# khaotik/DaNet-Tensorflow

Hardware: AMD Instinct MI355X
Metric: mixture-seconds/s (train step) (higher is better)
Workload: dtype f32; 1 GPU; cfg2: synthetic 8 kHz 2-spk, FFT 256/64 (129 bins), T=128, 3x300 BiLSTM, E=20, anchor estimator (A=6), dot-softmax, B=32/GPU; global_batch=32, parallelism=dp1, grad_allreduce_bytes=27619696, grad_allreduce_schedule=0

## Files before the change

danet-tensorflow_amd/_build.py:

```python
import collections
import glob
import os
import subprocess
import sys
from concurrent.futures import ThreadPoolExecutor

HERE = os.path.dirname(os.path.abspath(__file__))
CSRC = os.path.join(HERE, 'csrc')
INCLUDE = os.path.join(os.path.dirname(HERE), 'include')
ARCH = 'gfx950'
HIPCC = os.environ.get('HIPCC', '/opt/rocm/bin/hipcc')
FLAGS = ['--offload-arch=' + ARCH, '-O3', '-std=c++17', '-fPIC', '-fvisibility=hidden', '-I' + INCLUDE,
         '-I' + CSRC, '-Wno-unused-result']
FLAGS += os.environ.get('DANET_BUILD_DEFS', '').split()

Library = collections.namedtuple('Library', 'out src_dir headers')


def _extension(name, *more_headers):
    src_dir = os.path.join(CSRC, name)
    return Library(os.path.join(CSRC, 'libdanet_%s_hip.so' % name), src_dir,
                   (os.path.join(INCLUDE, 'danet_%s_hip.h' % name),) + more_headers)


def _shared(*names):
    return tuple(os.path.join(CSRC, n + '.h') for n in names)


CORE = Library(os.path.join(CSRC, 'libdanet_hip.so'), CSRC, (os.path.join(CSRC, '*.h'), os.path.join(INCLUDE, '*.h')))
CONV = _extension('conv', os.path.join(CSRC, 'conv', '*.h'), *_shared('ext_core'))
DROPOUT = _extension('dropout', *_shared('ext_core'))
PREP = _extension('prep', *_shared('ext_core'))
MIX = _extension('mix', *_shared('ext_core', 'ragged_rows', 'sumsq_f64'))
SPEED = _extension('speed', *_shared('ext_core', 'ragged_rows'))
LIBRARIES = (CORE, CONV, DROPOUT, PREP, MIX, SPEED)
LIB, CONV_LIB, DROPOUT_LIB, PREP_LIB, MIX_LIB, SPEED_LIB = (spec.out for spec in LIBRARIES)
REVERB = _extension('reverb', *_shared('ext_core', 'ragged_rows'))
LATER_LIBRARIES = (REVERB,)
REVERB_LIB = REVERB.out
METRIC = _extension('metric', *_shared('wave_metric', 'ext_core'))
NOISE = _extension('noise', *_shared('ext_core'))
LEVEL = _extension('level', *_shared('ext_core', 'ragged_rows'))
WAVLOSS = _extension('wavloss', *_shared('wave_metric', 'ext_core'))
GCLIP = _extension('gclip', *_shared('ext_core', 'adam_one', 'sumsq_f64'))
DPCL = _extension('dpcl', *_shared('ext_core'))
NEVAL = _extension('neval', *_shared('wave_metric', 'ext_core'))
EXTENSIONS = (METRIC, NOISE, LEVEL, WAVLOSS, GCLIP, DPCL, NEVAL)
STITCH = _extension('stitch', *_shared('ext_core'))
BSS = _extension('bss', *_shared('ext_core'))
STOI = _extension('stoi', *_shared('ext_core'))
PHASE = _extension('phase', *_shared('ext_core', 'wave_metric'))
ONLINE = _extension('online', *_shared('ext_core'))
CAUSAL = _extension('causal', *_shared('ext_core'))
MORE_EXTENSIONS = (STITCH, BSS, STOI, PHASE, ONLINE, CAUSAL)
METRIC_LIB = METRIC.out
NOISE_LIB = NOISE.out
LEVEL_LIB = LEVEL.out
WAVLOSS_LIB = WAVLOSS.out
GCLIP_LIB = GCLIP.out
DPCL_LIB = DPCL.out
NEVAL_LIB = NEVAL.out
STITCH_LIB = STITCH.out
BSS_LIB = BSS.out
STOI_LIB = STOI.out
PHASE_LIB = PHASE.out
ONLINE_LIB = ONLINE.out
CAUSAL_LIB = CAUSAL.out


def _sources(src_dir):
    return sorted(f for f in os.listdir(src_dir) if f.endswith(('.hip', '.cpp')))


def _compile(src_dir, src, bdir, force, hdr_m, defs=()):
    obj = os.path.join(bdir, os.path.splitext(src)[0] + '.o')
    sp = os.path.join(src_dir, src)
    if (not force and os.path.exists(obj)
            and os.path.getmtime(obj) > max(os.path.getmtime(sp), hdr_m)):
        return obj, False
    cmd = [HIPCC] + FLAGS + list(defs) + ['-c', sp, '-o', obj]
    if src.endswith('.hip'):
        cmd[1:1] = ['-x', 'hip']
    r = subprocess.run(cmd, capture_output=True, text=True)
    if r.returncode != 0:
        raise RuntimeError('hipcc failed for %s:\n%s\n%s' % (src, r.stdout, r.stderr))
    return obj, True


def _compile_all(src_dir, bdir, force, hdr_m, defs=()):
    os.makedirs(bdir, exist_ok=True)
    srcs = _sources(src_dir)
    with ThreadPoolExecutor(max_workers=min(8, len(srcs))) as ex:
        return list(ex.map(lambda s: _compile(src_dir, s, bdir, force, hdr_m, defs), srcs))


def _link(objs, out, src_dir):
    cmd = [HIPCC, '--offload-arch=' + ARCH, '-shared', '-fPIC',
           '-Wl,--version-script=' + os.path.join(src_dir, 'exports.map'), '-o', out] + objs
    r = subprocess.run(cmd, capture_output=True, text=True)
    if r.returncode != 0:
        raise RuntimeError('link failed:\n%s\n%s' % (r.stdout, r.stderr))


def _build_spec(spec, force, verbose):
    hdr_m = max((os.path.getmtime(h) for pattern in spec.headers for h in glob.glob(pattern)), default=0.0)
    res = _compile_all(spec.src_dir, os.path.join(spec.src_dir, 'build'), force, hdr_m)
    objs = [o for o, _ in res]
    rebuilt = any(r for _, r in res)
    if rebuilt or not os.path.exists(spec.out):
        _link(objs, spec.out, spec.src_dir)
    if verbose:
        print('%s: %s (%d objects, %s)' % (
            os.path.basename(spec.out), spec.out, len(objs), 'rebuilt' if rebuilt else 'up to date'))
    return spec.out


def _build_library(spec, force, verbose):
    return _build_spec(spec, force, verbose)


def build(force=False, verbose=True):
    for spec in LIBRARIES + LATER_LIBRARIES:
        _build_library(spec, force, verbose)
    return LIB


def build_all(force=False, verbose=True):
    build(force, verbose)
    for spec in EXTENSIONS + MORE_EXTENSIONS:
        _build_spec(spec, force, verbose)
    return [spec.out for spec in LIBRARIES + LATER_LIBRARIES + EXTENSIONS + MORE_EXTENSIONS]


def build_conv(force=False, verbose=True):
    return _build_library(CONV, force, verbose)


def build_dropout(force=False, verbose=True):
    return _build_library(DROPOUT, force, verbose)


def build_prep(force=False, verbose=True):
    return _build_library(PREP, force, verbose)


def build_mix(force=False, verbose=True):
    return _build_library(MIX, force, verbose)


def build_speed(force=False, verbose=True):
    return _build_library(SPEED, force, verbose)


def build_reverb(force=False, verbose=True):
    return _build_library(REVERB, force, verbose)


def build_metric(force=False, verbose=True):
    return _build_spec(METRIC, force, verbose)


def build_noise(force=False, verbose=True):
    return _build_spec(NOISE, force, verbose)


def build_level(force=False, verbose=True):
    return _build_spec(LEVEL, force, verbose)


def build_wavloss(force=False, verbose=True):
    return _build_spec(WAVLOSS, force, verbose)


def build_gclip(force=False, verbose=True):
    return _build_spec(GCLIP, force, verbose)


def build_dpcl(force=False, verbose=True):
    return _build_spec(DPCL, force, verbose)


def build_neval(force=False, verbose=True):
    return _build_spec(NEVAL, force, verbose)


def build_stitch(force=False, verbose=True):
    return _build_spec(STITCH, force, verbose)


def build_bss(force=False, verbose=True):
    return _build_spec(BSS, force, verbose)


def build_stoi(force=False, verbose=True):
    return _build_spec(STOI, force, verbose)


def build_phase(force=False, verbose=True):
    return _build_spec(PHASE, force, verbose)


def build_online(force=False, verbose=True):
    return _build_spec(ONLINE, force, verbose)


def build_causal(force=False, verbose=True):
    return _build_spec(CAUSAL, force, verbose)


def build_variant(name, defs):
    out = os.path.join(CSRC, 'libdanet_hip_%s.so' % name)
    res = _compile_all(CSRC, os.path.join(CSRC, 'build_' + name), True, 0.0, defs)
    _link([o for o, _ in res], out, CSRC)
    return out


def build_trace():
    return build_variant('trace', ['-DDANET_LSTM_TRACE'])


if __name__ == '__main__':
    if '--trace' in sys.argv:
        print(build_trace())
    elif '--variant' in sys.argv:
        i = sys.argv.index('--variant')
        print(build_variant(sys.argv[i + 1], sys.argv[i + 2:]))
    else:
        build_all(force='--force' in sys.argv)
```

danet-tensorflow_amd/_lib.py:

```python
import collections
import ctypes
import os
import threading

import torch

_CSRC = os.path.join(os.path.dirname(os.path.abspath(__file__)), 'csrc')

c_int, c_i64, c_f32, c_sz, c_p, c_u32 = (ctypes.c_int, ctypes.c_int64, ctypes.c_float,
                                         ctypes.c_size_t, ctypes.c_void_p, ctypes.c_uint32)
c_f64 = ctypes.c_double


class GemmPack(ctypes.Structure):
    _fields_ = [('src', c_p), ('stride_n', ctypes.c_longlong), ('stride_k', ctypes.c_longlong),
                ('N', c_int), ('K', c_int), ('out', c_p), ('out_bytes', c_sz)]


class GemmProblem(ctypes.Structure):
    _fields_ = [('A', c_p), ('lda', c_int), ('B', c_p), ('ldb', c_int), ('C', c_p), ('ldc', c_int),
                ('M', c_int), ('N', c_int), ('bias', c_p), ('beta', c_f32)]


PROTOTYPES = {
# ... 103 lines not shown
                                    c_u32, c_u32]),
}

PREP_PROTOTYPES = {
    'danet_prep_abi_version': (c_int, []),
    'danet_prep_last_error': (ctypes.c_char_p, []),
    'danet_prep_num_frames': (c_int, [c_i64, c_int, c_int]),
    'danet_prep_workspace_bytes': (c_sz, [c_int]),
    'danet_prep_stft_plan': (c_int, [c_p, c_int, c_p, c_p, c_sz]),
    'danet_prep_stft_batch': (c_int, [c_p, c_int, c_p, c_i64, c_p, c_int, c_int, c_int, c_int, c_int, c_p, c_p,
                                      c_p, c_i64]),
}

MIX_PROTOTYPES = {
    'danet_mix_abi_version': (c_int, []),
    'danet_mix_last_error': (ctypes.c_char_p, []),
    'danet_mix_workspace_bytes': (c_sz, [c_int, c_i64]),
    'danet_mix_power': (c_int, [c_p, c_int, c_p, c_i64, c_p, c_p, c_i64, c_p, c_p, c_sz]),
    'danet_mix_scale_c64': (c_int, [c_p, c_int, c_int, c_int, c_p, c_i64, c_p]),
}

SPEED_PROTOTYPES = {
    'danet_speed_abi_version': (c_int, []),
    'danet_speed_last_error': (ctypes.c_char_p, []),
    'danet_speed_out_len': (c_i64, [c_i64, c_int]),
    'danet_speed_resample': (c_int, [c_p, c_int, c_p, c_i64, c_p, c_p, c_p, c_i64]),
}

REVERB_PROTOTYPES = {
    'danet_reverb_abi_version': (c_int, []),
    'danet_reverb_last_error': (ctypes.c_char_p, []),
    'danet_reverb_apply': (c_int, [c_p, c_int, c_p, c_i64, c_p, c_p, c_int, c_p, c_i64]),
}

METRIC_PROTOTYPES = {
    'danet_metric_abi_version': (c_int, []),
    'danet_metric_last_error': (ctypes.c_char_p, []),
    'danet_metric_workspace_bytes': (c_sz, [c_int, c_int, c_int, c_int, c_int]),
    'danet_metric_synth': (c_int, [c_p, c_int, c_int, c_int, c_int, c_int, c_p, c_p, c_p, c_p]),
    'danet_metric_gram': (c_int, [c_p, c_int, c_int, c_i64, c_p, c_p]),
    'danet_metric_si_sdr': (c_int, [c_p, c_int, c_int, c_p, c_p, c_p, c_p]),
}

NOISE_PROTOTYPES = {
    'danet_noise_abi_version': (c_int, []),
    'danet_noise_last_error': (ctypes.c_char_p, []),
    'danet_noise_frontend_fwd': (c_int, [c_p, c_int, c_int, c_i64, c_p, c_p, c_p, c_p, c_p, c_p, c_p, c_p]),
}

LEVEL_PROTOTYPES = {
    'danet_level_abi_version': (c_int, []),
    'danet_level_last_error': (ctypes.c_char_p, []),
    'danet_level_workspace_bytes': (c_sz, [c_int, c_i64]),
    'danet_level_activity': (c_int, [c_p, c_int, c_p, c_i64, c_p, c_p, c_i64, c_f64, c_i64, c_p, c_p, c_p, c_sz]),
}

WAVLOSS_PROTOTYPES = {
    'danet_wavloss_abi_version': (c_int, []),
    'danet_wavloss_last_error': (ctypes.c_char_p, []),
    'danet_wavloss_fwd': (c_int, [c_p, c_int, c_int, c_p, c_p, c_p, c_p, c_p, c_p, c_p]),
    'danet_wavloss_bwd': (c_int, [c_p, c_int, c_int, c_int, c_int, c_int, c_p, c_p, c_p, c_p, c_p, c_p, c_p]),
}

GCLIP_PROTOTYPES = {
    'danet_gclip_abi_version': (c_int, []),
    'danet_gclip_last_error': (ctypes.c_char_p, []),
    'danet_gclip_partials': (c_int, [c_i64]),
    'danet_gclip_sumsq': (c_int, [c_p, c_i64, c_p, c_p, c_int]),
    'danet_gclip_adam_step': (c_int, [c_p, c_i64, c_p, c_p, c_p, c_p, c_f32, c_f32, c_f32, c_f32, c_f32, c_f32, c_int,
                                      c_f64, c_p, c_int, c_p]),
}

DPCL_PROTOTYPES = {
    'danet_dpcl_abi_version': (c_int, []),
    'danet_dpcl_last_error': (ctypes.c_char_p, []),
    'danet_dpcl_chunks': (c_int, [c_i64]),
    'danet_dpcl_workspace_bytes': (c_sz, [c_int, c_i64, c_int, c_int]),
    'danet_dpcl_stats': (c_int, [c_p, c_int, c_i64, c_int, c_int, c_p, c_p, c_p, c_sz]),
    'danet_dpcl_finalize': (c_int, [c_p, c_int, c_i64, c_int, c_int, c_p, c_sz, c_p, c_f32, c_p, c_p, c_p, c_p, c_p]),
    'danet_dpcl_bwd': (c_int, [c_p, c_int, c_i64, c_int, c_int, c_p, c_p, c_p, c_p, c_p, c_f32, c_p]),
}

NEVAL_PROTOTYPES = {
    'danet_neval_abi_version': (c_int, []),
    'danet_neval_last_error': (ctypes.c_char_p, []),
    'danet_neval_workspace_bytes': (c_sz, [c_int, c_int, c_int, c_int, c_int]),
    'danet_neval_synth': (c_int, [c_p, c_int, c_int, c_int, c_int, c_int, c_p, c_p, c_p, c_p, c_p, c_p]),
    'danet_neval_gram': (c_int, [c_p, c_int, c_int, c_i64, c_p, c_p]),
    'danet_neval_si_sdr': (c_int, [c_p, c_int, c_int, c_p, c_p, c_p, c_p]),
}

STITCH_PROTOTYPES = {
    'danet_stitch_abi_version': (c_int, []),
    'danet_stitch_last_error': (ctypes.c_char_p, []),
    'danet_stitch_chunks': (c_int, [c_int, c_int, c_int]),
    'danet_stitch_workspace_bytes': (c_sz, [c_int, c_int, c_int, c_int, c_int]),
    'danet_stitch_affinity': (c_int, [c_p, c_int, c_int, c_int, c_int, c_int, c_p, c_p, c_sz]),
    'danet_stitch_assign': (c_int, [c_p, c_int, c_int, c_int, c_int, c_int, c_p, c_sz, c_p, c_p]),
    'danet_stitch_merge': (c_int, [c_p, c_int, c_int, c_int, c_int, c_int, c_p, c_p, c_p, c_p, c_p]),
}

BSS_PROTOTYPES = {
    'danet_bss_abi_version': (c_int, []),
    'danet_bss_last_error': (ctypes.c_char_p, []),
    'danet_bss_workspace_bytes': (c_sz, [c_int, c_int, c_int]),
    'danet_bss_xcorr': (c_int, [c_p, c_int, c_int, c_i64, c_int, c_p, c_p, c_p, c_p]),
    'danet_bss_systems': (c_int, [c_p, c_int, c_int, c_int, c_p, c_p, c_p, c_p, c_p, c_p]),
    'danet_bss_chol_solve': (c_int, [c_p, c_int, c_int, c_int, c_p, c_p, c_p]),
    'danet_bss_finalize': (c_int, [c_p, c_int, c_int, c_int, c_p, c_p, c_p, c_p, c_p, c_p, c_p, c_int, c_int,
                                   c_p, c_p, c_p, c_p]),
}

STOI_PROTOTYPES = {
    'danet_stoi_abi_version': (c_int, []),
    'danet_stoi_last_error': (ctypes.c_char_p, []),
    'danet_stoi_workspace_bytes': (c_sz, [c_int, c_int, c_i64, c_int, c_int]),
    'danet_stoi_resample': (c_int, [c_p, c_int, c_int, c_i64, c_int, c_int, c_p, c_p, c_p]),
    'danet_stoi_frames': (c_int, [c_p, c_int, c_int, c_i64, c_p, c_p, c_p, c_p, c_p, c_p, c_p]),
    'danet_stoi_bands': (c_int, [c_p, c_int, c_int, c_i64, c_p, c_p, c_p, c_p, c_p, c_p, c_p]),
    'danet_stoi_segments': (c_int, [c_p, c_int, c_int, c_int, c_p, c_p, c_p]),
    'danet_stoi_finalize': (c_int, [c_p, c_int, c_int, c_int, c_p, c_p, c_p, c_int, c_int, c_p, c_p, c_p, c_p, c_p]),
}

PHASE_PROTOTYPES = {
    'danet_phase_abi_version': (c_int, []),
    'danet_phase_last_error': (ctypes.c_char_p, []),
    'danet_phase_workspace_bytes': (c_sz, [c_int, c_int, c_int, c_int, c_int]),
    'danet_phase_init': (c_int, [c_p, c_int, c_int, c_int, c_int, c_int, c_int, c_p, c_p, c_p, c_p, c_p]),
    'danet_phase_synth': (c_int, [c_p, c_int, c_int, c_int, c_int, c_int, c_p, c_p, c_p]),
    'danet_phase_project': (c_int, [c_p, c_int, c_int, c_int, c_int, c_int, c_p, c_p, c_p, c_p]),
}

ONLINE_PROTOTYPES = {
    'danet_online_abi_version': (c_int, []),
    'danet_online_last_error': (ctypes.c_char_p, []),
    'danet_online_state_bytes': (c_sz, [c_int, c_int]),
    'danet_online_init': (c_int, [c_p, c_int, c_int, c_int, c_p, c_p]),
    'danet_online_scan': (c_int, [c_p, c_int, c_int, c_int, c_int, c_int, c_int, c_f64, c_int, c_i64, c_f64, c_p, c_p,
                                  c_p, c_p]),
    'danet_online_separate': (c_int, [c_p, c_int, c_int, c_int, c_int, c_int, c_int, c_p, c_p, c_p, c_p]),
}

CAUSAL_PROTOTYPES = {
    'danet_causal_abi_version': (c_int, []),
    'danet_causal_last_error': (ctypes.c_char_p, []),
    'danet_causal_center_fwd': (c_int, [c_p, c_int, c_int, c_int, c_p, c_int, c_int, c_p, c_int, c_int, c_p]),
    'danet_causal_center_bwd': (c_int, [c_p, c_int, c_int, c_int, c_p, c_int, c_int, c_p, c_int, c_int]),
    'danet_causal_lstm_ws_bytes': (c_sz, [c_int, c_int, c_int, c_int]),
    'danet_causal_lstm_block': (c_int, [c_p, c_int, c_int, c_int, c_int, c_int, c_p, c_int, ctypes.POINTER(c_p),
                                        ctypes.POINTER(c_p), c_p, c_p, c_p, c_int, c_p, c_sz]),
    'danet_causal_project': (c_int, [c_p, c_int, c_int, c_int, c_p, c_int, c_p, c_int, c_p, c_int]),
}

Library = collections.namedtuple('Library', 'name so path_var handle_var prototypes abi prefix needs')
CONV_ABI_VERSION = DROPOUT_ABI_VERSION = PREP_ABI_VERSION = MIX_ABI_VERSION = SPEED_ABI_VERSION = 1
REVERB_ABI_VERSION = 1

CORE = Library('', 'libdanet_hip.so', 'LIB_PATH', '_lib', PROTOTYPES, 7, 'danet_',
               'the HIP extension is required')
CONV = Library('conv', 'libdanet_conv_hip.so', 'CONV_LIB_PATH', '_conv', CONV_PROTOTYPES, CONV_ABI_VERSION,
               'danet_conv_', 'the conv-bilstm-v1 encoder needs the HIP extension library')
DROPOUT = Library('dropout', 'libdanet_dropout_hip.so', 'DROPOUT_LIB_PATH', '_dropout', DROPOUT_PROTOTYPES,
                  DROPOUT_ABI_VERSION, 'danet_dropout_', 'DROPOUT_KEEP_PROB < 1 needs the HIP extension library')
PREP = Library('prep', 'libdanet_prep_hip.so', 'PREP_LIB_PATH', '_prep', PREP_PROTOTYPES, PREP_ABI_VERSION,
               'danet_prep_', 'the wavdir dataset needs the HIP extension library')
MIX = Library('mix', 'libdanet_mix_hip.so', 'MIX_LIB_PATH', '_mix', MIX_PROTOTYPES, MIX_ABI_VERSION,
              'danet_mix_', 'MIX_SNR_RANGE / MIX_LEVEL_RANGE need the HIP extension library')
SPEED = Library('speed', 'libdanet_speed_hip.so', 'SPEED_LIB_PATH', '_speed', SPEED_PROTOTYPES, SPEED_ABI_VERSION,
                'danet_speed_', 'SPEED_PERTURB_RANGE needs the HIP extension library')
REVERB = Library('reverb', 'libdanet_reverb_hip.so', 'REVERB_LIB_PATH', '_reverb', REVERB_PROTOTYPES,
                 REVERB_ABI_VERSION, 'danet_reverb_', 'REVERB_RT60_MAX needs the HIP extension library')
LIBRARIES = (CORE, CONV, DROPOUT, PREP, MIX)
ALL_LIBRARIES = LIBRARIES + (SPEED,)
LATER_LIBRARIES = (REVERB,)
METRIC_ABI_VERSION = 1
METRIC = Library('metric', 'libdanet_metric_hip.so', 'METRIC_LIB_PATH', '_metric', METRIC_PROTOTYPES,
                 METRIC_ABI_VERSION, 'danet_metric_', 'EVAL_SI_SDR needs the HIP extension library')
NOISE_ABI_VERSION = 1
NOISE = Library('noise', 'libdanet_noise_hip.so', 'NOISE_LIB_PATH', '_noise', NOISE_PROTOTYPES,
                NOISE_ABI_VERSION, 'danet_noise_', 'NOISE_DIR needs the HIP extension library')
LEVEL_ABI_VERSION = 1
LEVEL = Library('level', 'libdanet_level_hip.so', 'LEVEL_LIB_PATH', '_level', LEVEL_PROTOTYPES,
                LEVEL_ABI_VERSION, 'danet_level_', 'MIX_LEVEL_MEASURE needs the HIP extension library')
WAVLOSS_ABI_VERSION = 1
WAVLOSS = Library('wavloss', 'libdanet_wavloss_hip.so', 'WAVLOSS_LIB_PATH', '_wavloss', WAVLOSS_PROTOTYPES,
                  WAVLOSS_ABI_VERSION, 'danet_wavloss_', 'TRAIN_LOSS = "si-sdr" needs the HIP extension library')
GCLIP_ABI_VERSION = 1
GCLIP = Library('gclip', 'libdanet_gclip_hip.so', 'GCLIP_LIB_PATH', '_gclip', GCLIP_PROTOTYPES,
                GCLIP_ABI_VERSION, 'danet_gclip_', 'GRAD_CLIP_NORM needs the HIP extension library')
DPCL_ABI_VERSION = 1
DPCL = Library('dpcl', 'libdanet_dpcl_hip.so', 'DPCL_LIB_PATH', '_dpcl', DPCL_PROTOTYPES,
               DPCL_ABI_VERSION, 'danet_dpcl_', 'DPCL_WEIGHT needs the HIP extension library')
NEVAL_ABI_VERSION = 1
NEVAL = Library('neval', 'libdanet_neval_hip.so', 'NEVAL_LIB_PATH', '_neval', NEVAL_PROTOTYPES,
                NEVAL_ABI_VERSION, 'danet_neval_', 'NOISE_EVAL_DIR with EVAL_SI_SDR needs the HIP extension library')
STITCH_ABI_VERSION = 1
STITCH = Library('stitch', 'libdanet_stitch_hip.so', 'STITCH_LIB_PATH', '_stitch', STITCH_PROTOTYPES,
                 STITCH_ABI_VERSION, 'danet_stitch_', 'INFER_CHUNK_LEN needs the HIP extension library')
EXTENSIONS = (METRIC, NOISE, LEVEL, WAVLOSS, GCLIP, DPCL, NEVAL)
BSS_ABI_VERSION = 1
BSS = Library('bss', 'libdanet_bss_hip.so', 'BSS_LIB_PATH', '_bss', BSS_PROTOTYPES,
              BSS_ABI_VERSION, 'danet_bss_', 'EVAL_BSS_SDR needs the HIP extension library')
STOI_ABI_VERSION = 1
STOI = Library('stoi', 'libdanet_stoi_hip.so', 'STOI_LIB_PATH', '_stoi', STOI_PROTOTYPES,
               STOI_ABI_VERSION, 'danet_stoi_', 'EVAL_STOI needs the HIP extension library')
PHASE_ABI_VERSION = 1
PHASE = Library('phase', 'libdanet_phase_hip.so', 'PHASE_LIB_PATH', '_phase', PHASE_PROTOTYPES,
                PHASE_ABI_VERSION, 'danet_phase_', 'PHASE_REFINE_ITERS needs the HIP extension library')
ONLINE_ABI_VERSION = 1
ONLINE = Library('online', 'libdanet_online_hip.so', 'ONLINE_LIB_PATH', '_online', ONLINE_PROTOTYPES,
                 ONLINE_ABI_VERSION, 'danet_online_', 'the "online" estimator needs the HIP extension library')
CAUSAL_ABI_VERSION = 1
CAUSAL = Library('causal', 'libdanet_causal_hip.so', 'CAUSAL_LIB_PATH', '_causal', CAUSAL_PROTOTYPES,
                 CAUSAL_ABI_VERSION, 'danet_causal_', 'the lstm-causal encoder and streaming inference need the HIP '
                 'extension library')
MORE_EXTENSIONS = (STITCH, BSS, STOI, PHASE, ONLINE, CAUSAL)

LIB_PATH = os.environ.get('DANET_LIB_PATH') or os.path.join(_CSRC, CORE.so)
CONV_LIB_PATH = os.path.join(_CSRC, CONV.so)
DROPOUT_LIB_PATH = os.path.join(_CSRC, DROPOUT.so)
PREP_LIB_PATH = os.path.join(_CSRC, PREP.so)
MIX_LIB_PATH = os.path.join(_CSRC, MIX.so)
SPEED_LIB_PATH = os.path.join(_CSRC, SPEED.so)
REVERB_LIB_PATH = os.path.join(_CSRC, REVERB.so)
METRIC_LIB_PATH = os.path.join(_CSRC, METRIC.so)
NOISE_LIB_PATH = os.path.join(_CSRC, NOISE.so)
LEVEL_LIB_PATH = os.path.join(_CSRC, LEVEL.so)
WAVLOSS_LIB_PATH = os.path.join(_CSRC, WAVLOSS.so)
GCLIP_LIB_PATH = os.path.join(_CSRC, GCLIP.so)
DPCL_LIB_PATH = os.path.join(_CSRC, DPCL.so)
NEVAL_LIB_PATH = os.path.join(_CSRC, NEVAL.so)
STITCH_LIB_PATH = os.path.join(_CSRC, STITCH.so)
BSS_LIB_PATH = os.path.join(_CSRC, BSS.so)
STOI_LIB_PATH = os.path.join(_CSRC, STOI.so)
PHASE_LIB_PATH = os.path.join(_CSRC, PHASE.so)
ONLINE_LIB_PATH = os.path.join(_CSRC, ONLINE.so)
CAUSAL_LIB_PATH = os.path.join(_CSRC, CAUSAL.so)
_lib = _conv = _dropout = _prep = _mix = _speed = _reverb = _metric = _noise = _level = _wavloss = _gclip = _dpcl = None
_neval = _stitch = _bss = _stoi = _phase = _online = _causal = None
_lock = threading.Lock()


class DanetHipError(RuntimeError):
    pass


def _load(spec, loaded=None):
    g = globals()
    if g[spec.handle_var] is None:
        with _lock:
            if g[spec.handle_var] is None:
                path = g[spec.path_var]
                if not os.path.exists(path):
                    raise DanetHipError(
                        '%s not found at %s -- %s (there is no CPU fallback); build it with '
                        '`python -c "import __graft_entry__ as g; g.build()"`' % (spec.so, path, spec.needs))
                lib = ctypes.CDLL(path, mode=ctypes.RTLD_LOCAL)
                for name, (res, args) in spec.prototypes.items():
                    fn = getattr(lib, name)
                    fn.restype = res
                    fn.argtypes = args
                if getattr(lib, spec.prefix + 'abi_version')() != spec.abi:
                    raise DanetHipError('%s ABI version mismatch' % spec.so)
                g[spec.handle_var] = lib
                if loaded is not None:
                    loaded()
    return g[spec.handle_var]


def _check(spec, rc):
    msg = getattr(_load(spec), spec.prefix + 'last_error')()
    raise DanetHipError('%s error %d: %s' % (spec.so[:-3], rc, msg.decode() if msg else '?'))


def bytes_or_raise(nbytes, check):
    if nbytes == ctypes.c_size_t(-1).value:
        check(-1)
    return nbytes


def load():
    if _lib is not None:
        return _lib
    return _load(CORE, apply_env_options)


def load_conv():
    if _conv is not None:
        return _conv
    return _load(CONV)


def conv_check(rc):
    if rc != 0:
        _check(CONV, rc)


def conv_ws_bytes(op, desc):
    return bytes_or_raise(load_conv().danet_conv_workspace_bytes(op, ctypes.byref(desc)), conv_check)


def load_dropout():
    if _dropout is not None:
        return _dropout
    return _load(DROPOUT)


def dropout_check(rc):
    if rc != 0:
        _check(DROPOUT, rc)


def load_prep():
    if _prep is not None:
        return _prep
    return _load(PREP)


def prep_check(rc):
    if rc != 0:
        _check(PREP, rc)


def load_mix():
    if _mix is not None:
        return _mix
    return _load(MIX)


def mix_check(rc):
    if rc != 0:
        _check(MIX, rc)


def load_speed():
    if _speed is not None:
        return _speed
    return _load(SPEED)


def speed_check(rc):
    if rc != 0:
        _check(SPEED, rc)


def load_reverb():
    if _reverb is not None:
        return _reverb
    return _load(REVERB)


def reverb_check(rc):
    if rc != 0:
        _check(REVERB, rc)


def load_metric():
    if _metric is not None:
        return _metric
    return _load(METRIC)


def metric_check(rc):
    if rc != 0:
        _check(METRIC, rc)


def load_noise():
    if _noise is not None:
        return _noise
    return _load(NOISE)


def noise_check(rc):
    if rc != 0:
        _check(NOISE, rc)


def load_level():
    if _level is not None:
        return _level
    return _load(LEVEL)


def level_check(rc):
    if rc != 0:
        _check(LEVEL, rc)


def load_wavloss():
    if _wavloss is not None:
        return _wavloss
    return _load(WAVLOSS)


def wavloss_check(rc):
    if rc != 0:
        _check(WAVLOSS, rc)


def load_gclip():
    if _gclip is not None:
        return _gclip
    return _load(GCLIP)


def gclip_check(rc):
    if rc != 0:
        _check(GCLIP, rc)


def load_dpcl():
    if _dpcl is not None:
        return _dpcl
    return _load(DPCL)


def dpcl_check(rc):
    if rc != 0:
        _check(DPCL, rc)


def load_neval():
    if _neval is not None:
        return _neval
    return _load(NEVAL)


def neval_check(rc):
    if rc != 0:
        _check(NEVAL, rc)


def load_stitch():
    if _stitch is not None:
        return _stitch
    return _load(STITCH)


def stitch_check(rc):
    if rc != 0:
        _check(STITCH, rc)


def load_bss():
    if _bss is not None:
        return _bss
    return _load(BSS)


def bss_check(rc):
    if rc != 0:
        _check(BSS, rc)


def load_stoi():
    if _stoi is not None:
        return _stoi
    return _load(STOI)


def stoi_check(rc):
    if rc != 0:
        _check(STOI, rc)


def load_phase():
    if _phase is not None:
        return _phase
    return _load(PHASE)


def phase_check(rc):
    if rc != 0:
        _check(PHASE, rc)


def load_online():
    if _online is not None:
        return _online
    return _load(ONLINE)


def online_check(rc):
    if rc != 0:
        _check(ONLINE, rc)


def load_causal():
    if _causal is not None:
        return _causal
    return _load(CAUSAL)


def causal_check(rc):
    if rc != 0:
        _check(CAUSAL, rc)


_expert = None
_expert_seen = set()


def expert(name, default):
    global _expert
    if _expert is None:
        _expert = {}
        for item in os.environ.get('DANET_EXPERT', '').split(','):
            if item.strip():
                k, _, v = item.partition('=')
                _expert[k.strip().lower()] = v.strip()
    _expert_seen.add(name.lower())
    v = _expert.get(name.lower())
    if v is None:
        return default
    if isinstance(default, bool):
        return v not in ('0', 'false', 'no', '')
    return type(default)(v)


USER_OPTIONS = ('lstm_fwd_fused', 'lstm_spin_limit', 'lstm_fault_inject')


def option_names():
    lib = _lib
    return [lib.danet_option_name(i).decode() for i in range(lib.danet_option_count())]


def apply_env_options():
    lib = _lib
    lib.danet_reset_options()
    for name in option_names():
        v = os.environ.get('DANET_' + name.upper()) if name in USER_OPTIONS else None
        if v is None or v.strip() == '':
            v = expert(name, '')
        if v != '':
            check(lib.danet_set_option(name.encode(), int(v)))
    unknown = sorted(set(_expert or {}) - _expert_seen)
    if unknown:
        import warnings
        warnings.warn('DANET_EXPERT: unknown setting(s) %s (known: the lower-case constants of ops.py / model.py '
                      'that call _lib.expert(), and the library options %s)' % (unknown, option_names()))


def set_option(name, value):
    check(load().danet_set_option(name.encode(), int(value)))


def get_option(name):
    v = c_int(0)
    check(load().danet_get_option(name.encode(), ctypes.byref(v)))
    return v.value


def check(rc):
    if rc != 0:
        _check(CORE, rc)


(WS_ISTFT, WS_GEMM, WS_GEMM_STREAMK, WS_COLSUM, WS_LSTM, WS_ATTRACTOR_TRUTH, WS_ATTRACTOR_ANCHOR,
 WS_SEPARATE_BWD, WS_SEPARATE_PIT, WS_SEPARATE_PIT_RECORDS, WS_PIT_MSE, WS_CENTER_MEAN,
 WS_GEMM_X6, WS_GEMM_PACK, WS_GEMM_X6_TN, WS_SEPARATE_PIT_GRAD) = range(16)


def ws_bytes(op, *dims):
    arr = (c_i64 * len(dims))(*[int(d) for d in dims])
    return bytes_or_raise(load().danet_workspace_bytes(op, arr, len(dims)), check)


def ptr(t):
    if t is None:
        return None
    return t.data_ptr()


def stream():
    return torch.cuda.current_stream().cuda_stream


_ws = {}


def workspace(nbytes, device, tag=None):
    key = (device.index if device.index is not None else torch.cuda.current_device(),
           torch.cuda.current_stream().cuda_stream, tag)
    t = _ws.get(key)
    if t is None or t.numel() < nbytes:
        t = torch.zeros(max(int(nbytes), 1 << 20), dtype=torch.uint8, device=device)
        _ws[key] = t
    return t


_prof = None
_prof_only = None
_prof_on = True


def profile_start(only=None):
    global _prof, _prof_only
    if torch.cuda.is_available():
        prepare_timing(64)
    _prof = {}
    _prof_only = set(only) if only else None


def profile_enable(flag):
    global _prof_on
    _prof_on = bool(flag)


def profile_stop():
    global _prof
    p, _prof = _prof, None
    torch.cuda.synchronize()
    out = {}
    for label, evs in (p or {}).items():
        out[label] = (len(evs), sum(a.elapsed_time(b) for a, b in evs))
    return out


ATTACHED_LABELS = frozenset(('lstm_fwd', 'lstm_bwd'))
_aux_stream = None
_event_pool = []


def _timing_event():
    global _aux_stream
    if _event_pool:
        return _event_pool.pop()
    return _timing_event_new()


def prepare_timing(n=384):
    made = False
    while len(_event_pool) < n:
        _event_pool.append(_timing_event_new())
        made = True
    if made:
        torch.cuda.synchronize()


def _timing_event_new():
    global _aux_stream
    if _aux_stream is None:
        _aux_stream = torch.cuda.Stream()
    e = torch.cuda.Event(enable_timing=True)
    e.record(_aux_stream)
    return e


class timed(object):
    __slots__ = ('label', 'tag', 'a', 'b')

    def __init__(self, label, tag=None):
        self.label, self.tag = label, tag

    def __enter__(self):
        self.a = self.b = None
        if _prof is not None and _prof_on and (_prof_only is None or self.label in _prof_only):
            if self.label in ATTACHED_LABELS:
                self.a, self.b = _timing_event(), _timing_event()
                check(load().danet_next_launch_events(self.a.cuda_event, self.b.cuda_event))
            else:
                self.a = torch.cuda.Event(enable_timing=True)
                self.a.record()
        return self

    def __exit__(self, *exc):
        if self.a is not None and _prof is not None:
            b = self.b
            if b is None:
                b = torch.cuda.Event(enable_timing=True)
                b.record()
            _prof.setdefault(self.label, []).append((self.a, b))
            if self.tag:
                _prof.setdefault(self.label + ':' + self.tag, []).append((self.a, b))
        return False
```

danet-tensorflow_amd/csrc/gemm_x6.hip:

```cpp
#include "common.h"
#include <hip/hip_ext.h>
#include <atomic>
#include "danet_hip.h"
#include "options.h"

typedef __bf16 bf16x8 __attribute__((ext_vector_type(8)));
typedef uint32_t u32x4 __attribute__((ext_vector_type(4)));
typedef uint32_t u32x2 __attribute__((ext_vector_type(2)));

#define XBN 128
#define X6_OOB 0xfffffff0u
#define XBK 16

template <int MI> struct X6Geo {
  static constexpr int BM = 64 * MI;
  static constexpr int IMG = BM * XBK * 2;
  static constexpr int STAGE = 3 * IMG;
  static constexpr int LDC_T = XBN + 4;
  static constexpr int EPI = 32 * MI * LDC_T * 4;
  static constexpr int SMEM = 3 * STAGE > EPI ? 3 * STAGE : EPI;
  static constexpr int NS = 12 * MI;
  static constexpr int WG_PER_CU = MI == 2 ? 2 : 1;
};

// ... 749 lines not shown
      *reinterpret_cast<f32x4*>(o) = v;
    }
  }
}

template <bool RAGGED>
__global__ __launch_bounds__(256, 2) void gemm_x6_tn_kernel(X6TArgs g) {
  extern __shared__ __attribute__((aligned(16))) char xsm[];
  if ((int)blockIdx.x < g.ntail) {
    x6t_tail(g, (int)blockIdx.x, xsm);
    return;
  }
  const int tid = threadIdx.x, lane = tid & 63, wave = __builtin_amdgcn_readfirstlane(tid >> 6);
  const int wm = wave >> 1, wn = wave & 1;
  const int item = x6_xcd_item((int)blockIdx.x - g.ntail, (int)gridDim.x - g.ntail);
  const int z = item / g.tiles;
  const int t = item % g.tiles;
  int pi = 0;
#pragma unroll
  for (int i = 1; i < X6T_MAX_PROBLEMS; ++i)
    if (i < g.nprob && t >= g.p[i].tile0) pi = i;
  const X6TProblem& q = g.p[pi];
  const int tl = t - q.tile0;
  const int m0 = (tl / q.tiles_n) * 128, n0 = (tl % q.tiles_n) * 128;
  const int M = q.Mmain, N = q.N, K = g.K;

  const int nkt = (K + 15) / 16;
  const int per = (nkt + g.splitk - 1) / g.splitk;
  const int kt0 = z * per, kt1 = min(nkt, kt0 + per);

  X6TCtx c;
  {
    const float* ab = q.A + m0;
    const float* bb = q.B + n0;
    c.rsa = __builtin_amdgcn_make_buffer_rsrc(const_cast<float*>(ab), 0, (int)(((size_t)(K - 1) * q.lda + ((M - m0 + 3) & ~3)) * 4), 0x00020000);
    c.rsb = __builtin_amdgcn_make_buffer_rsrc(const_cast<float*>(bb), 0, (int)(((size_t)(K - 1) * q.ldb + ((N - n0 + 3) & ~3)) * 4), 0x00020000);
  }
  c.lda = q.lda; c.ldb = q.ldb; c.K = K; c.kt1 = kt1; c.mrem = M - m0; c.nrem = N - n0;
  const int kr = lane >> 4, mq = lane & 15;
  c.krow = 4 * wave + kr;
  c.mq4 = 4 * mq;
#pragma unroll
  for (int li = 0; li < 4; ++li) {
    const int col = c.mq4 + (li & 1) * 64;
    c.lvo[li] = col < (li < 2 ? c.mrem : c.nrem) ? (unsigned)(c.krow * (li < 2 ? c.lda : c.ldb) + col) * 4u : X6_OOB;
  }
  c.woff = (wave * 8 + (mq >> 2)) * 128 + ((kr + (mq >> 2)) & 3) * 32 + (mq & 3) * 8;
  {
    const int i16 = lane & 15, mbit = (lane >> 4) & 1, kh = lane >> 5;
#pragma unroll
    for (int i = 0; i < 2; ++i) {
      const int ba = (wm * 64 + i * 32 + 16 * mbit) >> 4, bb = (wn * 64 + i * 32 + 16 * mbit) >> 4;
      c.roffa[i] = (2 * kh * 8 + ba) * 128 + (((i16 >> 2) + ba) & 3) * 32 + (i16 & 3) * 8;
      c.roffb[i] = (2 * kh * 8 + bb) * 128 + (((i16 >> 2) + bb) & 3) * 32 + (i16 & 3) * 8;
    }
  }
  const int fi = lane & 31, kb = lane >> 5;

  f32x16 acc[2][2];
#pragma unroll
  for (int i = 0; i < 2; ++i)
#pragma unroll
    for (int j = 0; j < 2; ++j)
#pragma unroll
      for (int r = 0; r < 16; ++r) acc[i][j][r] = 0.f;

  if (kt0 < kt1) {
    f32x4 R0[4], R1[4];
    bf16x8 faA[3][2], fbA[3][2], faB[3][2], fbB[3][2];
    x6t_load_tile<RAGGED>(c, kt0, R0); x6t_load_tile<RAGGED>(c, kt0 + 1, R1);
    x6t_store_tile(xsm, c, R0); x6t_store_tile(xsm + TSTAGE, c, R1);
    x6t_load_tile<RAGGED>(c, kt0 + 2, R0); x6t_load_tile<RAGGED>(c, kt0 + 3, R1);
    __syncthreads();
    x6t_frags(xsm, c, faA, fbA);
    int kt = kt0, srd = 1, swr = 2;
#define X6T_STEP(SRD, SWR, R, FAC, FBC, FAN, FBN)                                                    \
    { x6t_step<RAGGED, SRD, SWR>(c, xsm, kt, srd, swr, acc, R, FAC, FBC, FAN, FBN);                  \
      __syncthreads();                                                                               \
      ++kt; }
#define X6T_STEP_RT(R, FAC, FBC, FAN, FBN)                                                           \
    { x6t_step<RAGGED, -1, -1>(c, xsm, kt, srd, swr, acc, R, FAC, FBC, FAN, FBN);                    \
      __syncthreads();                                                                               \
      ++kt; srd = swr; swr = swr == 2 ? 0 : swr + 1; }
    while (kt + 5 < kt1) {
      X6T_STEP(1, 2, R0, faA, fbA, faB, fbB)
      X6T_STEP(2, 0, R1, faB, fbB, faA, fbA)
      X6T_STEP(0, 1, R0, faA, fbA, faB, fbB)
      X6T_STEP(1, 2, R1, faB, fbB, faA, fbA)
      X6T_STEP(2, 0, R0, faA, fbA, faB, fbB)
      X6T_STEP(0, 1, R1, faB, fbB, faA, fbA)
    }
    while (kt + 1 < kt1) {
      X6T_STEP_RT(R0, faA, fbA, faB, fbB)
      X6T_STEP_RT(R1, faB, fbB, faA, fbA)
    }
    if (kt < kt1) X6T_STEP_RT(R0, faA, fbA, faB, fbB)
#undef X6T_STEP
#undef X6T_STEP_RT
  }

  const bool sliced = g.splitk > 1;
  float* __restrict__ dst = sliced ? g.slab + (size_t)z * g.slab_stride + q.slab_off : q.C;
  const int ldc = sliced ? N : q.ldc;
  const float beta = sliced ? 0.f : q.beta;
  const bool vec = (ldc % 4 == 0) && (((uintptr_t)dst & 15) == 0) && (n0 + 128 <= N);
  if (vec) {
    float* ct = reinterpret_cast<float*>(xsm);
    constexpr int LDC_T = 132;
#pragma unroll
    for (int half = 0; half < 2; ++half) {
      __syncthreads();
      if (wm == half) {
#pragma unroll
        for (int i = 0; i < 2; ++i)
#pragma unroll
          for (int j = 0; j < 2; ++j)
#pragma unroll
            for (int r = 0; r < 16; ++r)
              ct[(i * 32 + (r & 3) + 8 * (r >> 2) + 4 * kb) * LDC_T + wn * 64 + j * 32 + fi] = acc[i][j][r];
      }
      __syncthreads();
#pragma unroll
      for (int it = 0; it < 8; ++it) {
        const int rr = (tid >> 5) + 8 * it, c4 = tid & 31;
        const int row = m0 + half * 64 + rr;
        if (row < M) {
          f32x4* o = reinterpret_cast<f32x4*>(dst + (size_t)row * ldc + n0 + c4 * 4);
          f32x4 v = *reinterpret_cast<const f32x4*>(&ct[rr * LDC_T + c4 * 4]);
          if (beta != 0.f) v += *o;
          *o = v;
        }
      }
    }
    return;
  }
#pragma unroll
  for (int i = 0; i < 2; ++i)
#pragma unroll
    for (int j = 0; j < 2; ++j) {
      const int col = n0 + wn * 64 + j * 32 + fi;
#pragma unroll
      for (int r = 0; r < 16; ++r) {
        const int row = m0 + wm * 64 + i * 32 + (r & 3) + 8 * (r >> 2) + 4 * kb;
        if (row < M && col < N) {
          float* o = dst + (size_t)row * ldc + col;
          *o = acc[i][j][r] + (beta != 0.f ? *o : 0.f);
        }
      }
    }
}

__global__ __launch_bounds__(256) void gemm_x6_tn_reduce_kernel(X6TArgs g) {
  const X6TProblem& q = g.p[blockIdx.y];
  const int M = q.M, N = q.N, ldc = q.ldc;
  const float beta = q.beta;
  const float* __restrict__ slab = g.slab + q.slab_off;
  const int64_t n4 = (int64_t)M * N / 4;
  for (int64_t i = (int64_t)blockIdx.x * 256 + threadIdx.x; i < n4; i += (int64_t)gridDim.x * 256) {
    f32x4 v = reinterpret_cast<const f32x4*>(slab)[i];
    for (int s = 1; s < g.splitk; ++s) v += reinterpret_cast<const f32x4*>(slab + (size_t)s * g.slab_stride)[i];
    const int64_t e = i * 4;
    f32x4* o = reinterpret_cast<f32x4*>(q.C + (size_t)(e / N) * ldc + (e % N));
    if (beta != 0.f) v += *o;
    *o = v;
  }
}

#ifdef X6T_FORCE_S
static int x6t_splitk(int tiles, int K) { return tiles >= 100 ? X6T_FORCE_S : x6_slices(tiles, cdiv(K, 16), 16, 8); }
#else
static int x6t_splitk(int tiles, int K) { return x6_slices(tiles, cdiv(K, 16), 16, 8, 0.045); }
#endif
static int x6t_main_rows(int M, int N) {
  const int tail = M % 128;
  return (M > 128 && tail >= 1 && tail <= X6T_TAIL_MAX && N % 4 == 0) ? M - tail : M;
}
size_t dn_ws_gemm_x6_tn(long long sum_mn, int tiles, int K) {
  const int s = x6t_splitk(tiles, K);
  return s > 1 ? (size_t)s * (size_t)sum_mn * sizeof(float) : 0;
}

extern "C" int danet_gemm_x6_tn_grouped(danet_stream_t stream_, int K, int nprob, const danet_gemm_problem_t* probs,
                                        void* ws, size_t ws_bytes) {
  hipStream_t stream = (hipStream_t)stream_;
  DANET_CHECK_ARG(probs && nprob >= 1 && nprob <= X6T_MAX_PROBLEMS, "gemm_x6_tn: 1..%d problems", X6T_MAX_PROBLEMS);
  DANET_CHECK_ARG(K > 0, "gemm_x6_tn: non-positive K %d", K);
  X6TArgs g;
  int tiles = 0;
  long long sum_mn = 0;
  bool slicable = true, ragged = false;
  for (int i = 0; i < nprob; ++i) {
    const danet_gemm_problem_t& q = probs[i];
    DANET_CHECK_ARG(q.M > 0 && q.N > 0 && q.A && q.B && q.C, "gemm_x6_tn: bad problem %d", i);
    DANET_CHECK_ARG(q.bias == nullptr && (q.beta == 0.f || q.beta == 1.f), "gemm_x6_tn: no bias; beta 0 or 1");
    DANET_CHECK_ARG(q.lda >= q.M && q.ldb >= q.N && q.ldc >= q.N, "gemm_x6_tn: leading dimension too small");
    if (q.lda % 4 || q.ldb % 4 || ((((uintptr_t)q.A | (uintptr_t)q.B)) & 15) != 0) {
      danet_set_error("gemm_x6_tn: lda / ldb must be multiples of 4 and A / B 16-byte aligned (problem %d)", i);
      return DANET_ERR_UNSUPPORTED;
    }
    DANET_CHECK_ARG((long long)K * q.lda < (1ll << 29) && (long long)K * q.ldb < (1ll << 29),
                    "gemm_x6_tn: an operand spans 2 GiB or more");
    X6TProblem& p = g.p[i];
    p.A = q.A; p.B = q.B; p.C = q.C; p.lda = q.lda; p.ldb = q.ldb; p.ldc = q.ldc; p.M = q.M; p.N = q.N;
    p.beta = q.beta;
    p.Mmain = ((((uintptr_t)q.C) & 15) == 0 && q.ldc % 4 == 0) ? x6t_main_rows(q.M, q.N) : q.M;
    p.tiles_n = cdiv(q.N, 128);
    p.tile0 = tiles;
    p.slab_off = sum_mn;
    tiles += cdiv(p.Mmain, 128) * p.tiles_n;
    sum_mn += (long long)q.M * q.N;
    ragged = ragged || (p.Mmain % 2 != 0) || (q.N % 2 != 0);
    slicable = slicable && q.N % 4 == 0 && q.ldc % 4 == 0 && (((uintptr_t)q.C) & 15) == 0 && ((long long)q.M * q.N) % 4 == 0;
  }
  for (int i = nprob; i < X6T_MAX_PROBLEMS; ++i) g.p[i] = g.p[0];
  g.nprob = nprob; g.K = K; g.tiles = tiles;
  int s = slicable ? x6t_splitk(tiles, K) : 1;
  g.splitk = s;
  g.slab_stride = sum_mn;
  g.slab = (float*)ws;
  g.ntail = 0;
  for (int i = 0; i < nprob; ++i)
    if (g.p[i].Mmain < g.p[i].M) g.ntail += cdiv(g.p[i].N, 64) * s;
  if (s > 1) {
    const size_t need = (size_t)s * (size_t)sum_mn * sizeof(float);
    if (!ws || ws_bytes < need || ((uintptr_t)ws & 15) != 0) {
      danet_set_error("gemm_x6_tn: workspace %zu < %zu (or not 16-B aligned)", ws_bytes, need);
      return DANET_ERR_WORKSPACE;
    }
  }
  static std::atomic<unsigned long long> done[2];
  dim3 grid((unsigned)(tiles * s + g.ntail)), block(256);
  if (ragged) {
    DANET_CHECK_HIP(x6_set_lds((const void*)gemm_x6_tn_kernel<true>, X6T_SMEM_BYTES, done[1]));
    gemm_x6_tn_kernel<true><<<grid, block, X6T_SMEM_BYTES, stream>>>(g);
  } else {
    DANET_CHECK_HIP(x6_set_lds((const void*)gemm_x6_tn_kernel<false>, X6T_SMEM_BYTES, done[0]));
    gemm_x6_tn_kernel<false><<<grid, block, X6T_SMEM_BYTES, stream>>>(g);
  }
  DANET_CHECK_LAUNCH();
  if (s > 1) {
    long long most = 0;
    for (int i = 0; i < nprob; ++i) most = max(most, (long long)probs[i].M * probs[i].N / 4);
    dim3 rgrid((unsigned)min((long long)1024, (most + 255) / 256), (unsigned)nprob);
    gemm_x6_tn_reduce_kernel<<<rgrid, block, 0, stream>>>(g);
    DANET_CHECK_LAUNCH();
  }
  return DANET_OK;
}
```

danet-tensorflow_amd/csrc/lstm.hip:

```cpp
#include "common.h"
#include "options.h"
#include <hip/hip_ext.h>
#include <atomic>
#include <type_traits>
#include <stdlib.h>

void dn_take_launch_events(hipEvent_t* start, hipEvent_t* stop);
#define DN_LAUNCH_EV(K_, GRID_, BLOCK_, LDS_, STREAM_, ARGS_)                                        \
  do {                                                                                               \
    if (ev_start || ev_stop)                                                                         \
      hipExtLaunchKernelGGL(K_, dim3(GRID_), dim3(BLOCK_), LDS_, STREAM_, ev_start, ev_stop, 0, ARGS_); \
    else K_<<<GRID_, BLOCK_, LDS_, STREAM_>>>(ARGS_);                                                \
  } while (0)

#define LSTM_UNITS_FWD 8
#define SPIN_LIMIT (1u << 20)
#define FWD_CH 5
#define SENTINEL 0xFFFFFFFFu

#define RLX_AGENT __ATOMIC_RELAXED, __HIP_MEMORY_SCOPE_AGENT

typedef unsigned v4u __attribute__((__vector_size__(16)));

__device__ __forceinline__ v4u load_sc1_b128(__amdgpu_buffer_rsrc_t r, unsigned off) {
// ... 1197 lines not shown
      dp += gstep;
    }
    if constexpr (!SHADOW) { gp += gstep; cp += cstep; dyp += ystep; }
    TRACE(5);
  }
  shadow_store(T - 1);
  if constexpr (PRE) { if (othr) db_add(); }
  if (a.dbslab != nullptr && tw == 0) {
    float* dbt = &atile[SSTORE ? (T & 1) * ATILE : 0];
    __syncthreads();
    if (othr) {
      float* ap = &dbt[orow * LDA + oj];
      ap[0] = dbacc[0]; ap[U] = dbacc[1]; ap[2 * U] = dbacc[2]; ap[3 * U] = dbacc[3];
    }
    __syncthreads();
    if (tid < 4 * U) {
      float v = 0.f;
#pragma unroll
      for (int rr = 0; rr < 16; ++rr) v += dbt[rr * LDA + tid];
      const int gate = tid / U, j = tid % U;
      if (u0 + j < H) a.dbslab[(size_t)cl * (4 * H) + gate * H + u0 + j] = v;
    }
  }
}

__global__ __launch_bounds__(256) void lstm_db_reduce_kernel(
    const float* __restrict__ dbslab, float* db0, float* db1, int G, int H4, float beta) {
  const int dir = blockIdx.y;
  float* db = dir ? db1 : db0;
  const int q4 = H4 / 4;
  for (int j = blockIdx.x * 256 + threadIdx.x; j < q4; j += gridDim.x * 256) {
    f32x4 v = {0.f, 0.f, 0.f, 0.f};
    for (int g = 0; g < G; ++g)
      v += reinterpret_cast<const f32x4*>(dbslab + (size_t)(dir * G + g) * H4)[j];
    f32x4* o = reinterpret_cast<f32x4*>(db) + j;
    if (beta != 0.f) v += *o;
    *o = v;
  }
}

__global__ __launch_bounds__(256) void multi_fill_kernel(FillArgs a) {
  fill_share(a, (unsigned long long)blockIdx.x * 256 + threadIdx.x, (unsigned long long)gridDim.x * 256);
}

struct FillList {
  FillArgs a;
  FillList() { a.nseg = 0; }
  bool full() const { return a.nseg >= FILL_MAXSEG; }
  void add(void* p, size_t bytes, unsigned value) {
    a.ptr[a.nseg] = p; a.n16[a.nseg] = bytes / 16; a.value[a.nseg] = value; ++a.nseg;
  }
  hipError_t launch(hipStream_t stream) {
    unsigned long long tot = 0;
    for (int i = 0; i < a.nseg; ++i) tot += a.n16[i];
    unsigned long long blocks = (tot + 256 * 4 - 1) / (256 * 4);
    if (blocks > 2048) blocks = 2048;
    if (blocks < 1) blocks = 1;
    multi_fill_kernel<<<(unsigned)blocks, 256, 0, stream>>>(a);
    return hipGetLastError();
  }
};

struct LstmPlan { int MT, G, P, KP, NW, UN; size_t lds; };

int dn_num_cus() {
  static std::atomic<int> n{0};
  int c = n.load(std::memory_order_relaxed);
  if (c) return c;
  int dev = 0, v = 0;
  if (hipGetDevice(&dev) == hipSuccess &&
      hipDeviceGetAttribute(&v, hipDeviceAttributeMultiprocessorCount, dev) == hipSuccess && v > 0) {
    n.store(v, std::memory_order_relaxed);
    return v;
  }
  (void)hipGetLastError();
  return 256;
}

static LstmPlan make_plan(int B, int H, int ndir) {
  LstmPlan pl;
  pl.UN = LSTM_UNITS_FWD;
  pl.P = cdiv(H, pl.UN);
  pl.KP = cdiv(H, 16) * 16;
  pl.MT = (ndir * cdiv(B, 16) * pl.P > dn_num_cus()) ? 2 : 1;
  if (B > 4) {
    const int want = danet_opt(OPT_LSTM_FWD_UN);
    const bool fits12 = ndir * cdiv(B, 16) * cdiv(H, 12) <= dn_num_cus();
    if ((want == 12 || (want != 8 && pl.MT == 2)) && fits12) {
      pl.UN = 12; pl.P = cdiv(H, 12); pl.MT = 1;
    }
  }
  pl.G = cdiv(B, 16 * pl.MT);
  pl.NW = 4;
  { const int ngw = cdiv(pl.KP / 16, pl.NW), nbw = (ngw + 1) / 2;
    pl.lds = (((size_t)pl.NW * 16 * pl.MT * (4 * pl.UN + 1) + 3) & ~(size_t)3) * sizeof(float) +
             (size_t)pl.NW * (nbw > 3 ? nbw - 3 : 0) * 3 * (4 * pl.UN / 16) * 64 * 16; }
  return pl;
}

struct RsPlan { bool ok; int U, G, P, S, NT, NTW, NI, D; size_t ring_bytes; };
static RsPlan make_rs_plan(int B, int H, int ndir, int U) {
  RsPlan r;
  r.U = U; r.G = cdiv(B, 16); r.P = cdiv(H, U);
  r.NT = cdiv(r.P * U, 16); r.D = 3;
  r.NI = cdiv(r.P, 512 / (4 * U));
  const int ncl = ndir * r.G;
  int smax = dn_num_cus() / (ncl * r.P);
  if (smax > r.NT) smax = r.NT;
  r.S = smax;
  for (int sv = 1; sv <= smax; ++sv)
    if (cdiv(r.NT, sv) <= 8) { r.S = sv; break; }
  { const int es = danet_opt(OPT_LSTM_BWD_S);
    if (es >= 1 && es <= smax) r.S = es; }
  r.NTW = r.S > 0 ? cdiv(cdiv(r.NT, r.S), 8) : 99;
  r.ring_bytes = (size_t)r.D * ncl * r.P * r.NT * 1024;
  r.ok = (H % 4 == 0) && smax >= 1 && r.NTW <= 5 && r.NI <= RS_NI_MAX &&
         r.ring_bytes < 0xFFFFFFF0ull;
  return r;
}
static RsPlan choose_rs_plan(int B, int H, int ndir) {
  RsPlan none; none.ok = false; none.ring_bytes = 0;
  const int pin = danet_opt(OPT_LSTM_BWD_U);
  if (!pin && H > 384) {
    const RsPlan r = make_rs_plan(B, H, ndir, 16);
    if (r.ok) return r;
  }
  RsPlan best = none;
  int best_cost = 1 << 30;
  for (int U = 8; U <= 32; U *= 2) {
    if (pin && pin != U) continue;
    RsPlan r = make_rs_plan(B, H, ndir, U);
    if (!r.ok) continue;
    const int cost = cdiv(cdiv(r.NT, r.S), 4) * U;
    if (cost < best_cost) { best = r; best_cost = cost; }
  }
  return best;
}
static size_t ring_offset(int T) { return (64 + TRACE_BYTES(T) + 255) / 256 * 256; }
static unsigned spin_limit_env() {
  const long v = danet_opt(OPT_LSTM_SPIN_LIMIT);
  return v >= 256 ? (unsigned)v : SPIN_LIMIT;
}
static int fault_env() { return danet_opt(OPT_LSTM_FAULT_INJECT) == 1; }

size_t dn_ws_lstm(int T, int B, int H, int ndir) {
  size_t ring = 0;
  for (int U = 8; U <= 32; U *= 2) {
    RsPlan r = make_rs_plan(B, H, ndir, U);
    if (r.ok && r.ring_bytes > ring) ring = r.ring_bytes;
  }
  return align_up(ring_offset(T) + ring, 256) + align_up((size_t)ndir * cdiv(B, 16) * 4 * H * sizeof(float), 256);
}

static int lstm_check_common(int T, int B, int H, int ndir, void* ws, size_t ws_bytes) {
  DANET_CHECK_ARG(T > 0 && B > 0 && H > 0, "lstm: non-positive shape");
  DANET_CHECK_ARG(ndir == 1 || ndir == 2, "lstm: ndir must be 1 or 2");
  if (H % 4 != 0) {
    danet_set_error("lstm: H=%d must be a multiple of 4", H);
    return DANET_ERR_UNSUPPORTED;
  }
  if (!ws || ((uintptr_t)ws & 15) != 0 || ws_bytes < dn_ws_lstm(T, B, H, ndir)) {
    danet_set_error("lstm: workspace too small or not 16-B aligned");
    return DANET_ERR_WORKSPACE;
  }
  return DANET_OK;
}

static int prefill_fwd_segments(FillList& fl, hipStream_t stream, int T, int B, int ldy, int n,
                                float* const* ypads, void* const* wss) {
  const size_t blk = (size_t)B * ldy * sizeof(float);
  for (int i = 0; i < n; ++i) {
    DANET_CHECK_ARG(ypads[i] && ((uintptr_t)ypads[i] & 15) == 0, "lstm_prefill: ypad %d null / misaligned", i);
    if (fl.a.nseg + 4 > FILL_MAXSEG) { DANET_CHECK_HIP(fl.launch(stream)); fl = FillList(); }
    if (wss && wss[i]) fl.add(wss[i], 64 + TRACE_BYTES(T), 0u);
    fl.add((char*)ypads[i] + blk, (size_t)T * blk, SENTINEL);
    fl.add(ypads[i], blk, 0u);
    fl.add((char*)ypads[i] + (size_t)(T + 1) * blk, blk, 0u);
  }
  return DANET_OK;
}

static int prefill_bwd_segments(FillList& fl, hipStream_t stream, int T, const RsPlan& rs, int n,
                                void* const* wss) {
  for (int i = 0; i < n; ++i) {
    DANET_CHECK_ARG(wss[i] && ((uintptr_t)wss[i] & 15) == 0, "lstm_prefill: ws %d null / misaligned", i);
    if (fl.a.nseg + 2 > FILL_MAXSEG) { DANET_CHECK_HIP(fl.launch(stream)); fl = FillList(); }
    fl.add(wss[i], 64 + TRACE_BYTES(T), 0u);
    fl.add((char*)wss[i] + ring_offset(T), rs.ring_bytes, 1u);
  }
  return DANET_OK;
}

extern "C" int danet_lstm_fwd_prefill(danet_stream_t stream_, int T, int B, int ldy, int n,
                                      float* const* ypads, void* const* wss) {
  hipStream_t stream = (hipStream_t)stream_;
  DANET_CHECK_ARG(T > 0 && B > 0 && ldy > 0 && ldy % 4 == 0 && n > 0 && ypads, "lstm_fwd_prefill: bad argument");
  FillList fl;
  const int rc = prefill_fwd_segments(fl, stream, T, B, ldy, n, ypads, wss);
  if (rc) return rc;
  if (fl.a.nseg) DANET_CHECK_HIP(fl.launch(stream));
  return DANET_OK;
}

extern "C" int danet_lstm_train_prefill(danet_stream_t stream_, int T, int B, int H, int ndir, int ldy,
                                        int n, float* const* ypads, void* const* fwd_wss,
                                        void* const* bwd_wss) {
  hipStream_t stream = (hipStream_t)stream_;
  DANET_CHECK_ARG(T > 0 && B > 0 && H > 0 && (ndir == 1 || ndir == 2) && ldy > 0 && ldy % 4 == 0 && n > 0 &&
                  ypads && bwd_wss, "lstm_train_prefill: bad argument");
  const RsPlan rs = choose_rs_plan(B, H, ndir);
  if (!rs.ok) {
    danet_set_error("lstm_train_prefill: B=%d H=%d outside the reduce-scatter geometry", B, H);
    return DANET_ERR_UNSUPPORTED;
  }
  FillList fl;
  int rc = prefill_fwd_segments(fl, stream, T, B, ldy, n, ypads, fwd_wss);
  if (rc) return rc;
  rc = prefill_bwd_segments(fl, stream, T, rs, n, bwd_wss);
  if (rc) return rc;
  if (fl.a.nseg) DANET_CHECK_HIP(fl.launch(stream));
  return DANET_OK;
}

extern "C" int danet_encoder_prologue(danet_stream_t stream_, int B, int T, int D, const float* in,
                                      int in_layout, int ld_in, float* out, int out_layout, int ld_out,
                                      float* mean, int H, int ndir, int ldy, int n, float* const* ypads,
                                      void* const* fwd_wss, void* const* bwd_wss) {
  hipStream_t stream = (hipStream_t)stream_;
  DANET_CHECK_ARG(T > 0 && B > 0 && H > 0 && (ndir == 1 || ndir == 2) && ldy > 0 && ldy % 4 == 0 && n > 0 &&
                  ypads, "encoder_prologue: bad argument");
  FillList fl;
  int rc;
  const bool one = 4 * n + (bwd_wss ? 2 * n : 0) <= FILL_MAXSEG;
  if (bwd_wss) {
    const RsPlan rs = choose_rs_plan(B, H, ndir);
    if (!rs.ok) {
      danet_set_error("encoder_prologue: B=%d H=%d outside the reduce-scatter geometry", B, H);
      return DANET_ERR_UNSUPPORTED;
    }
    rc = prefill_fwd_segments(fl, stream, T, B, ldy, n, ypads, fwd_wss);
    if (rc) return rc;
    rc = prefill_bwd_segments(fl, stream, T, rs, n, bwd_wss);
    if (rc) return rc;
  } else {
    rc = prefill_fwd_segments(fl, stream, T, B, ldy, n, ypads, fwd_wss);
    if (rc) return rc;
  }
  bool taken = false;
  rc = dn_center(stream, B, T, D, in, in_layout, ld_in, out, out_layout, ld_out, mean,
                 one && fl.a.nseg ? &fl.a : nullptr, &taken);
  if (rc) return rc;
  if (!taken && fl.a.nseg) DANET_CHECK_HIP(fl.launch(stream));
  return DANET_OK;
}

extern "C" int danet_lstm_fwd(danet_stream_t stream_, int T, int B, int H, int ndir,
                              const float* gx_f, const float* gx_b,
                              const float* Wh_f, const float* Wh_b, int ldw,
                              float* ypad, int ldy, float* gates_f, float* gates_b,
                              float* cell_f, float* cell_b, void* ws, size_t ws_bytes,
                              int32_t* status, int flags) {
  hipEvent_t ev_start, ev_stop;
  dn_take_launch_events(&ev_start, &ev_stop);
  hipStream_t stream = (hipStream_t)stream_;
  int rc = lstm_check_common(T, B, H, ndir, ws, ws_bytes);
  if (rc) return rc;
  DANET_CHECK_ARG(gx_f && Wh_f && ypad && gates_f && cell_f, "lstm_fwd: null pointer");
  DANET_CHECK_ARG(ndir == 1 || (gx_b && Wh_b && gates_b && cell_b), "lstm_fwd: null bwd pointer");
  DANET_CHECK_ARG(ldy >= ndir * H && ldy % 4 == 0 && ldw >= 4 * H, "lstm_fwd: bad ld");
  DANET_CHECK_ARG(((uintptr_t)ypad & 15) == 0, "lstm_fwd: ypad must be 16-B aligned");
  DANET_CHECK_ARG((size_t)(T + 2) * B * ldy * 4 < 0xFFFFFFF0ull, "lstm_fwd: ypad > 4 GiB");
  LstmPlan pl = make_plan(B, H, ndir);
  if (pl.lds > 160 * 1024) {
    danet_set_error("lstm_fwd: H=%d needs %zu B LDS", H, pl.lds);
    return DANET_ERR_UNSUPPORTED;
  }
  const int nblk = ndir * pl.G * pl.P;
  if (nblk > dn_num_cus()) {
    danet_set_error("lstm_fwd: %d workgroups exceed the %d CUs", nblk, dn_num_cus());
    return DANET_ERR_UNSUPPORTED;
  }
  LstmFwdArgs a;
  a.gx[0] = gx_f; a.gx[1] = gx_b; a.Wh[0] = Wh_f; a.Wh[1] = Wh_b;
  a.gates[0] = gates_f; a.gates[1] = gates_b; a.cell[0] = cell_f; a.cell[1] = cell_b;
  a.ypad = ypad; a.status = status ? (int*)status : (int*)ws;
  a.spin_limit = spin_limit_env(); a.fault = fault_env();
  a.T = T; a.B = B; a.H = H; a.ndir = ndir; a.ldy = ldy; a.ldw = ldw;
  a.P = pl.P; a.G = pl.G; a.KP = pl.KP;
  a.xmap = (danet_opt(OPT_LSTM_XMAP) >= 0 ? danet_opt(OPT_LSTM_XMAP) : 1);
  const size_t blk = (size_t)B * ldy * sizeof(float);
  if (!(flags & DANET_LSTM_PREFILLED)) {
    FillList fl;
    fl.add(ws, 64 + TRACE_BYTES(T), 0u);
    fl.add((char*)ypad + blk, (size_t)T * blk, SENTINEL);
    fl.add(ypad, blk, 0u);
    fl.add((char*)ypad + (size_t)(T + 1) * blk, blk, 0u);
    DANET_CHECK_HIP(fl.launch(stream));
  }
#define LAUNCH_FWD(MTV, NWV, UNV)                                                    \
  do {                                                                               \
    DANET_CHECK_HIP(hipFuncSetAttribute((const void*)lstm_fwd_kernel<MTV, NWV, UNV>,  \
        hipFuncAttributeMaxDynamicSharedMemorySize, (int)pl.lds));                   \
    DN_LAUNCH_EV((lstm_fwd_kernel<MTV, NWV, UNV>), nblk, 64 * NWV, pl.lds, stream, a); \
  } while (0)
  if (B <= 4 && H <= 16 * FWD_CH * 4 && danet_opt(OPT_LSTM_FWD_SMALL) != 0) {
    const size_t lds = ((size_t)pl.KP * 32 + (size_t)4 * 4 * 33) * sizeof(float);
// ... 194 lines not shown
```

danet-tensorflow_amd/csrc/workspace.cpp:

```cpp
#include <stddef.h>
#include <stdint.h>
#include "danet_hip.h"

extern "C" void danet_set_error(const char* fmt, ...);

size_t dn_ws_istft(int n_sig, int T, int N, int S);
size_t dn_ws_gemm(int M, int N, int K);
size_t dn_ws_gemm_streamk(int M, int N, int K);
size_t dn_ws_colsum(int M, int N);
size_t dn_ws_lstm(int T, int B, int H, int ndir);
size_t dn_ws_attractor_truth(int B, int C, int64_t N, int E);
size_t dn_ws_attractor_anchor(int B, int C, int64_t N, int E, int A);
size_t dn_ws_separate_bwd(int B, int C, int64_t N, int E);
size_t dn_ws_separate_pit(int B, int C, int64_t N, int E);
size_t dn_ws_separate_pit_records(int B, int64_t N);
size_t dn_ws_pit_mse(int B, int C, int64_t N);
int dn_center_mean_elems(int B);
size_t dn_ws_gemm_x6(int M, int N, int K1, int K2);
size_t dn_ws_gemm_pack(int N, int K);
size_t dn_ws_gemm_x6_tn(long long sum_mn, int tiles, int K);
size_t dn_ws_separate_pit_grad(int B, int C, int64_t N, int E);

extern "C" size_t danet_workspace_bytes(int op, const int64_t* d, int n) {
  static const int kDims[DANET_WS_COUNT] = {4, 3, 3, 2, 4, 4, 5, 4, 4, 2, 3, 1, 4, 2, 3, 4};
  if (op < 0 || op >= DANET_WS_COUNT || !d || n != kDims[op]) {
    danet_set_error("workspace_bytes: op %d takes %d dims, got %d", op,
                    (op >= 0 && op < DANET_WS_COUNT) ? kDims[op] : -1, n);
    return (size_t)-1;
  }
  for (int i = 0; i < n; ++i)
    if (d[i] < 0 || (d[i] > 0x7fffffff && !(i == 2 && op >= DANET_WS_ATTRACTOR_TRUTH) &&
                     !(i == 1 && op == DANET_WS_SEPARATE_PIT_RECORDS) &&
                     !(i == 0 && op == DANET_WS_GEMM_X6_TN))) {
      danet_set_error("workspace_bytes: dim %d of op %d out of range", i, op);
      return (size_t)-1;
    }
  switch (op) {
    case DANET_WS_ISTFT: return dn_ws_istft((int)d[0], (int)d[1], (int)d[2], (int)d[3]);
    case DANET_WS_GEMM: return dn_ws_gemm((int)d[0], (int)d[1], (int)d[2]);
    case DANET_WS_GEMM_STREAMK: return dn_ws_gemm_streamk((int)d[0], (int)d[1], (int)d[2]);
    case DANET_WS_COLSUM: return dn_ws_colsum((int)d[0], (int)d[1]);
    case DANET_WS_LSTM: return dn_ws_lstm((int)d[0], (int)d[1], (int)d[2], (int)d[3]);
    case DANET_WS_ATTRACTOR_TRUTH: return dn_ws_attractor_truth((int)d[0], (int)d[1], d[2], (int)d[3]);
    case DANET_WS_ATTRACTOR_ANCHOR:
      return dn_ws_attractor_anchor((int)d[0], (int)d[1], d[2], (int)d[3], (int)d[4]);
    case DANET_WS_SEPARATE_BWD: return dn_ws_separate_bwd((int)d[0], (int)d[1], d[2], (int)d[3]);
    case DANET_WS_SEPARATE_PIT: return dn_ws_separate_pit((int)d[0], (int)d[1], d[2], (int)d[3]);
    case DANET_WS_SEPARATE_PIT_RECORDS: return dn_ws_separate_pit_records((int)d[0], d[1]);
    case DANET_WS_PIT_MSE: return dn_ws_pit_mse((int)d[0], (int)d[1], d[2]);
    case DANET_WS_CENTER_MEAN: return (size_t)dn_center_mean_elems((int)d[0]) * sizeof(float);
    case DANET_WS_GEMM_X6: return dn_ws_gemm_x6((int)d[0], (int)d[1], (int)d[2], (int)d[3]);
    case DANET_WS_GEMM_PACK: return dn_ws_gemm_pack((int)d[0], (int)d[1]);
    case DANET_WS_GEMM_X6_TN: return dn_ws_gemm_x6_tn((long long)d[0], (int)d[1], (int)d[2]);
    case DANET_WS_SEPARATE_PIT_GRAD: return dn_ws_separate_pit_grad((int)d[0], (int)d[1], d[2], (int)d[3]);
  }
  return (size_t)-1;
}
```

danet-tensorflow_amd/model.py:

```python
import math
import os

import numpy as np
import torch

from .hparams import hparams
from . import _lib, ops
from . import modules
from . import ozers
from . import dist


class Model(object):

    def __init__(self, name='BaseModel', device=None, seed=1337, grad_schedule=None):
        self.grad_schedule = str(grad_schedule if grad_schedule is not None else
                                 os.environ.get('DANET_OVERLAP_ALLREDUCE', 'auto'))
        assert self.grad_schedule in ('0', 'tail', '1', 'auto'), self.grad_schedule
        self.schedule_decision = None
        self._auto = self.grad_schedule == 'auto'
        if self._auto:
            self.grad_schedule = '0'
        self.name = name
        self.device = torch.device(device if device is not None else
# ... 374 lines not shown

    def _auto_tick(self):
        n = self.step_count
        if n == self.AUTO_DECIDE_AT - 3:
            self._auto_ev = torch.cuda.Event(enable_timing=True)
            self._auto_ev.record()
        if n < self.AUTO_DECIDE_AT or self._auto_ev is None:
            return
        end = torch.cuda.Event(enable_timing=True)
        end.record()
        end.synchronize()
        step_ms = dist.allreduce_max_scalar(self._auto_ev.elapsed_time(end) / 3.0, self.device)
        ar_ms = dist.measure_allreduce_ms(self._grad_store.numel(), self.device)
        mode = dist.choose_schedule(ar_ms, step_ms)
        self.schedule_decision = dict(schedule=mode, allreduce_ms=round(ar_ms, 4), step_ms=round(step_ms, 4),
                                      ratio=round(ar_ms / step_ms, 5), threshold=dist.TAIL_RATIO,
                                      bucket_bytes=4 * self._grad_store.numel(), decided_at_step=n,
                                      world=dist.world_size())
        self._auto, self._auto_ev = False, None
        self._install_schedule(mode)

    @property
    def _early_adam(self):
        return self._early_adam_on

    @_early_adam.setter
    def _early_adam(self, on):
        self._early_adam_on = bool(on)
        if on and not self._early_hooked:
            ops.add_grad_ready_hook(self._grad_ready)
            self._early_hooked = True

    def _grad_ready(self, tag, params):
        if self.grad_clip_norm is not None:
            return
        if tag[0] != 'rest' or not self._early_adam or not self._in_step or self._early is not None:
            return
        rng = [self._offs.get(p.data_ptr()) for p in params]
        if any(r is None for r in rng):
            return
        if dist.is_dist():
            if not isinstance(self._buckets, dist.TailOverlap):
                return
            self._buckets.wait_launched()
        ranges = dist._complement(rng, self._flat_grad.numel())
        self.ozer.step(self.step_count + 1, self.learn_rate, clip=hparams.GRAD_CLIP_THRES,
                       grad_scale=1.0 / dist.world_size(), zero_grad=not self.keep_grads,
                       ranges=ranges)
        ops.repack_weights(self.device)
        self._early = (ranges, torch.cuda.current_stream(self.device))
        self.early_steps += 1

    def dropout_spec(self, keep):
        if self._dropout is None or self._dropout.keep != float(keep):
            self._dropout = ops.DropoutSpec(keep, self.seed & 0xffffffff, dist.rank(),
                                            self.step_base + self.step_count)
        return self._dropout

    def forward(self, s_src_signals, with_valid=False, with_train=True, fuse_heads=False,
                s_dropout_keep=1.0):
        B, E = hparams.BATCH_SIZE, hparams.EMBED_SIZE
        eps = float(hparams.EPS)
        if self._noise is None:
            fe = ops.frontend(s_src_signals)
        else:
            fe = ops.noise_frontend(s_src_signals, *self._noise)
        self._dropout = None
        if s_dropout_keep < 1.0:
            s_embed = self.encoder(fe['mix_log'], s_dropout_keep)
        else:
            s_embed = self.encoder(fe['mix_log'])
        s_embed_flat = s_embed.reshape(B, -1, E)
        out = dict(embed=s_embed, input=s_src_signals)
        phasor = fe['phasor']
        if with_train:
            s_attractors = self.estimator(
                s_embed, s_src_pwr=fe['src_pwr'], s_mix_pwr=fe['mix_pwr'])
            act = getattr(self.separator, 'ACT', None)
            if self.dpcl_weight is not None:
                ops.unshare_dembed(s_attractors)
            if self.train_loss == 'si-sdr':
                s_sep_pwr = self.separator(fe['mix_pwr'], s_attractors, s_embed_flat)
                loss, loss_idx = ops.si_sdr_loss(s_src_signals, s_sep_pwr, phasor)
                with torch.no_grad():
                    _mse, perms, idx, snr = ops.pit_mse_loss(
                        s_src_signals, s_sep_pwr.detach(), phasor, mode=0, eps=eps)
                out.update(attrs=s_attractors, sep_pwr=s_sep_pwr, loss=loss, SNR=snr,
                           perm_idx=idx, perms=perms, loss_perm_idx=loss_idx)
            elif fuse_heads and act is not None and not hparams.DEBUG and not with_valid:
                loss, perms, idx, snr = ops.separate_pit_loss(
                    fe['mix_pwr'], s_attractors, s_embed_flat, s_src_signals, phasor, act,
                    mode=0, eps=eps)
                out.update(attrs=s_attractors, loss=loss, SNR=snr, perm_idx=idx, perms=perms)
            else:
                s_sep_pwr = self.separator(fe['mix_pwr'], s_attractors, s_embed_flat)
                loss, perms, idx, snr = ops.pit_mse_loss(
                    s_src_signals, s_sep_pwr, phasor, mode=0, eps=eps)
                out.update(attrs=s_attractors, sep_pwr=s_sep_pwr, loss=loss, SNR=snr,
                           perm_idx=idx, perms=perms)
            if self.dpcl_weight is not None:
                out['loss'], out['dpcl'] = ops.dpcl_loss(s_embed_flat, fe['src_pwr'], out['loss'], self.dpcl_weight)
        if with_valid:
            if self.using_same_method and with_train:
                s_vattr, s_vsep = out['attrs'], out['sep_pwr']
            else:
                if self.valid_estimator.USE_TRUTH:
                    s_vattr = self.valid_estimator(
                        s_embed, s_src_pwr=fe['src_pwr'], s_mix_pwr=fe['mix_pwr'])
                else:
                    s_vattr = self.valid_estimator(s_embed, s_mix_pwr=fe['mix_pwr'])
                s_vsep = self._separate(fe['mix_pwr'], s_vattr, s_embed_flat)
            vloss, perms, vidx, vsnr = ops.pit_mse_loss(
                s_src_signals, s_vsep, phasor, mode=1, eps=eps)
            out.update(valid_attrs=s_vattr, sep_pwr_valid=s_vsep, valid_loss=vloss,
                       valid_SNR=vsnr, valid_perm_idx=vidx, perms=perms)
        out['phasor'] = phasor
        out['mix_pwr'] = fe['mix_pwr']
        return out

    def forward_noisy(self, s_src_signals, s_noise, s_noise_gain=None, **kw):
        self._noise = (s_noise, s_noise_gain)
        try:
            return self.forward(s_src_signals, **kw)
        finally:
            self._noise = None

    def debug_fetch(self, s_src_signals):
        with torch.no_grad():
            o = self.forward(s_src_signals)
            res = dict(embed=o['embed'], attrs=o['attrs'], input=s_src_signals,
                       output=ops.reattach_phase(o['sep_pwr'], o['phasor'], o['perm_idx']))
            for mod in (self.encoder, self.separator, self.estimator):
                res.update(getattr(mod, 'debug_fetches', {}) or {})
        return res

    def train_step(self, s_src_signals, sync_metrics=True, s_noise=None, s_noise_gain=None):
        ops.poll_status(self.device)
        if not self._grads_clean:
            self._flat_grad.zero_()
        chain = ops.heads_chain()
        chain.__enter__()
        try:
            if s_noise is None:
                out = self.forward(s_src_signals, fuse_heads=self.fuse_heads,
                                   s_dropout_keep=float(hparams.DROPOUT_KEEP_PROB))
            else:
                out = self.forward_noisy(s_src_signals, s_noise, s_noise_gain, fuse_heads=self.fuse_heads,
                                         s_dropout_keep=float(hparams.DROPOUT_KEEP_PROB))
        except BaseException:
            chain.__exit__(None, None, None)
            ops.drop_lazy(self.device)
            raise
        self._early, self._in_step = None, True
        self._grads_clean = False
        try:
            with ops.fast_backward():
                out['loss'].backward(self._one)
                ops.join_deferred()
                if self._buckets is not None:
                    grad_scale = self._buckets.finish()
                else:
                    grad_scale = dist.allreduce_grads_(
                        self._grad_store if dist.is_dist() else self._flat_grad)
        finally:
            self._in_step = False
            chain.__exit__(None, None, None)
            ops.join_deferred()
        self.step_count += 1
        ranges, early_stream = None, None
        if self._early is not None:
            early, early_stream = self._early
            ranges = dist._complement(early, self._flat_grad.numel())
            self._early = None
        norm_out = None
        if self.grad_clip_norm is None:
            self.ozer.step(self.step_count, self.learn_rate, clip=hparams.GRAD_CLIP_THRES,
                           grad_scale=grad_scale, zero_grad=not self.keep_grads, ranges=ranges)
        else:
            self._gclip_partials = ops.grad_sumsq(self._flat_grad, self._gclip_partials)
            norm_out = torch.empty(2, dtype=torch.float64, device=self.device)
            self.ozer.step(self.step_count, self.learn_rate, clip=hparams.GRAD_CLIP_THRES,
                           grad_scale=grad_scale, zero_grad=not self.keep_grads, max_norm=self.grad_clip_norm,
                           partials=self._gclip_partials, norm_out=norm_out)
        ops.repack_weights(self.device)
        if early_stream is not None:
            torch.cuda.current_stream(self.device).wait_stream(early_stream)
        self._grads_clean = not self.keep_grads
        ops.step_done(self.device)
        if self._auto:
            self._auto_tick()
        res = dict(loss=out['loss'].detach(), SNR=out['SNR'], LR=self.learn_rate)
        if self.dpcl_weight is not None:
            res['DPCL'] = out['dpcl']
        if norm_out is not None:
            res.update(grad_norm=norm_out[0], clip_coef=norm_out[1])
        return res

    def collectives_per_step(self):
        if not dist.is_dist():
            return 0
        return {'0': 1, 'tail': 2}.get(self.grad_schedule,
                                       1 + hparams.NUM_LSTM_LAYERS + 1)

    def valid_step(self, s_src_signals, s_noise=None, s_noise_gain=None):
        ops.poll_status(self.device)
        if s_noise is not None:
            with torch.no_grad():
                out = self.forward_noisy(s_src_signals, s_noise, s_noise_gain, with_valid=True, with_train=False)
                res = dict(loss=out['valid_loss'], SNR=out['valid_SNR'])
                if self.eval_si_sdr:
                    est = ops.reattach_phase(out['sep_pwr_valid'], out['phasor'])
                    res['SI-SDR'], res['SI-SDRi'], res['nSNR'] = ops.si_sdr_noisy(
                        s_src_signals, est, s_noise, s_noise_gain)[:3]
            ops.step_done(self.device, collective_consistent=not dist.is_dist())
            return res
        with torch.no_grad():
            out = self.forward(s_src_signals, with_valid=True, with_train=False)
            res = dict(loss=out['valid_loss'], SNR=out['valid_SNR'])
            wav = None
            if self.eval_si_sdr:
                est = self._refined(ops.reattach_phase(out['sep_pwr_valid'], out['phasor']), s_src_signals)
                if self.eval_bss is None and not self.eval_stoi:
                    res['SI-SDR'], res['SI-SDRi'] = ops.si_sdr(s_src_signals, est)[:2]
                else:
                    res['SI-SDR'], res['SI-SDRi'], _, _, wav = ops.si_sdr_wav(s_src_signals, est)
            elif self.eval_bss is not None or self.eval_stoi:
                est = self._refined(ops.reattach_phase(out['sep_pwr_valid'], out['phasor']), s_src_signals)
                if self.eval_bss is not None and self.eval_stoi:
                    wav = ops.synth_wav(s_src_signals, est)
            if self.eval_bss is not None:
                res['SDR'], res['SIR'], res['SAR'], res['SDRi'] = ops.bss_eval(
                    s_src_signals, est, self.eval_bss, wav=wav)[:4]
            if self.eval_stoi:
                res['STOI'], res['ESTOI'], res['STOIi'], res['ESTOIi'] = ops.stoi_eval(s_src_signals, est, wav=wav)[:4]
        ops.step_done(self.device, collective_consistent=not dist.is_dist())
        return res

    def _refined(self, est, mixrows):
        if self.phase_refine is None:
            return est
        return ops.phase_refine(est, mixrows, self.phase_refine)

    def infer(self, s_mixed_signals):
        if self.stream_block is not None:
            return self._infer_stream(s_mixed_signals)
        if self.infer_chunk is not None:
            if s_mixed_signals.shape[0] != 1:
                raise ValueError('INFER_CHUNK_LEN is set: infer takes one recording at a time (got a batch of %d)'
                                 % s_mixed_signals.shape[0])
            if s_mixed_signals.shape[1] > self.infer_chunk[0]:
                return self.infer_long(s_mixed_signals)
        B, E = hparams.BATCH_SIZE, hparams.EMBED_SIZE
        ops.poll_status(self.device)
        with torch.no_grad():
            fe = ops.frontend(s_mixed_signals[:, None].contiguous())
            s_embed = self.encoder(fe['mix_log'])
            s_attr = self.valid_estimator(s_embed, s_mix_pwr=fe['mix_pwr'])
            s_sep = self._separate(fe['mix_pwr'], s_attr, s_embed.reshape(B, -1, E))
            res = self._refined(ops.reattach_phase(s_sep, fe['phasor']), s_mixed_signals[:, None])
        ops.step_done(self.device, collective_consistent=not dist.is_dist())
        return res

    def _infer_stream(self, s_mixed_signals):
        if hparams.BATCH_SIZE > ops.CAUSAL_MAX_B:
            raise ValueError('INFER_STREAM_BLOCK needs BATCH_SIZE <= %d when infer runs (got %d)'
                             % (ops.CAUSAL_MAX_B, hparams.BATCH_SIZE))
        n, T = self.stream_block, s_mixed_signals.shape[1]
        ops.poll_status(self.device)
        stream = self.open_stream(s_mixed_signals.shape[0])
        parts = [stream.push(s_mixed_signals[:, t:t + n]) for t in range(0, T, n)]
        parts.append(stream.flush())
        ops.step_done(self.device, collective_consistent=not dist.is_dist())
        return torch.cat(parts, dim=2)

    def infer_chunks(self, s_chunks):
        G = self.infer_chunk[2] if self.infer_chunk is not None else 16
        n, L, F = s_chunks.shape
        C, E = hparams.MAX_N_SIGNAL, hparams.EMBED_SIZE
        mags = torch.empty(n, C, L, F, device=self.device)
        phasor = torch.empty(n, L, F, 2, device=self.device)
        ops.poll_status(self.device)
        batch_size = hparams.BATCH_SIZE
        try:
            with torch.no_grad():
                for g0 in range(0, n, G):
                    g = min(G, n - g0)
                    hparams.BATCH_SIZE = g
                    fe = ops.frontend(s_chunks[g0:g0 + g, None].contiguous())
                    s_embed = self.encoder(fe['mix_log'])
                    s_attr = self.valid_estimator(s_embed, s_mix_pwr=fe['mix_pwr'])
                    mags[g0:g0 + g] = self.separator(fe['mix_pwr'], s_attr, s_embed.reshape(g, -1, E))
                    phasor[g0:g0 + g] = fe['phasor']
        finally:
            hparams.BATCH_SIZE = batch_size
        ops.step_done(self.device, collective_consistent=not dist.is_dist())
        return mags, phasor

    def infer_long(self, s_mixed_signals):
        L, V, _G = self.infer_chunk
        T = s_mixed_signals.shape[1]
        assert s_mixed_signals.shape[0] == 1 and T > L, s_mixed_signals.shape
        starts = ops.stitch_plan(T, L, V)
        s_chunks = torch.stack([s_mixed_signals[0, s:s + L] for s in starts])
        mags, phasor = self.infer_chunks(s_chunks)
        return self._refined(ops.stitch(mags, phasor, T, V)[None], s_mixed_signals[:, None])

    def set_learn_rate(self, lr):
        self.learn_rate = float(lr)

    def get_learn_rate(self):
        return self.learn_rate

    def check_status(self):
        ops.check_status(self.device)

    def status_words(self):
        return self._grad_store[:4]

    def zero_grad(self):
        self._flat_grad.zero_()
        self._grads_clean = True

    def reset_state(self):
        return

    def save_params(self, filename, step=None):
        save_dir = os.path.dirname(os.path.abspath(filename))
        if not os.path.exists(save_dir):
            os.makedirs(save_dir)
        if step is not None:
# ... 136 lines not shown
```

danet-tensorflow_amd/ops.py:

```python
import ctypes
import itertools
import math

import numpy as np
import torch

from . import _lib
from ._lib import ptr, check


def _L():
    return _lib.load()


def _f32(t):
    assert t.is_cuda and t.dtype == torch.float32, (t.device, t.dtype)
    return t


def _ws(nbytes, dev):
    w = _lib.workspace(nbytes, dev)
    return w, w.numel()


# ... 16 lines not shown
                stop_event.attached = True
        return C
    need = _lib.ws_bytes(_lib.WS_GEMM, M, N, K)
    w, wn = _ws(need, C.device)
    with _lib.timed('gemm_f32', tag):
        check(L.danet_gemm_f32(_lib.stream(), int(transA), int(transB), M, N, K,
                                  ptr(_f32(A)), lda, ptr(_f32(B)), ldb, ptr(_f32(C)), ldc,
                                  ptr(bias), float(beta), ptr(w), wn, int(max_workgroups)))
    return C


def gemm_kcat(A1, lda1, B1, ldb1, K1, A2, lda2, B2, ldb2, K2, C, M, N, ldc,
              transA=False, transB=False, bias=None, beta=0.0, tag=None, streamk=False,
              stop_event=None):
    L = _L()
    if streamk and K1 % 16 == 0:
        w = _lib.workspace(_lib.ws_bytes(_lib.WS_GEMM_STREAMK, M, N, K1 + K2), C.device,
                           tag='gemm_sk')
        with _lib.timed('gemm_f32', tag):
            if stop_event is not None:
                stop_event.arm()
            check(L.danet_gemm_f32_streamk_kcat(_lib.stream(), int(transA), int(transB), M, N,
                                                K1, ptr(_f32(A1)), lda1, ptr(_f32(B1)), ldb1,
                                                K2, ptr(_f32(A2)), lda2, ptr(_f32(B2)), ldb2,
                                                ptr(_f32(C)), ldc, ptr(bias), float(beta),
                                                ptr(w), w.numel()))
            if stop_event is not None:
                stop_event.attached = True
        return C
    gemm(A1, B1, C, M, N, K1, lda1, ldb1, ldc, transA=transA, transB=transB, bias=bias, beta=beta,
         tag=tag)
    gemm(A2, B2, C, M, N, K2, lda2, ldb2, ldc, transA=transA, transB=transB, beta=1.0, tag=tag)
    return C


GEMM_X6 = int(__import__('os').environ.get('DANET_GEMM_X6', '3'))


class _PackedWeight(object):
    __slots__ = ('W', 'N', 'K', 'sn', 'sk', 'lo', 'hi', 'out', 'stale', 'version', 'unused')

    def __init__(self, W, N, K, sn, sk):
        self.W, self.N, self.K, self.sn, self.sk = W, N, K, sn, sk
        self.lo = W.data_ptr()
        self.hi = self.lo + 4 * ((N - 1) * sn + (K - 1) * sk + 1)
        self.out = torch.empty(_lib.ws_bytes(_lib.WS_GEMM_PACK, N, K), dtype=torch.uint8,
                               device=W.device)
        self.stale, self.version, self.unused = True, -1, 0


_packs = {}


def _pack_now(pws):
    arr = (_lib.GemmPack * len(pws))()
    for i, pw in enumerate(pws):
        arr[i].src, arr[i].stride_n, arr[i].stride_k = pw.W.data_ptr(), pw.sn, pw.sk
        arr[i].N, arr[i].K = pw.N, pw.K
        arr[i].out, arr[i].out_bytes = pw.out.data_ptr(), pw.out.numel()
    check(_L().danet_gemm_pack_weights(_lib.stream(), len(pws), arr))
    for pw in pws:
        pw.stale, pw.version = False, pw.W._version


def packed_weight(W, N, K, sn, sk):
    reg = _packs.setdefault(_dev_key(W.device), {})
    key = (W.data_ptr(), N, K, sn, sk)
    pw = reg.get(key)
    if pw is None:
        pw = reg[key] = _PackedWeight(W, N, K, sn, sk)
    pw.unused = 0
    if pw.stale or pw.version != W._version:
        _pack_now([pw])
    return pw.out


def weights_written(t):
    reg = _packs.get(_dev_key(t.device))
    if reg:
        lo = t.data_ptr()
        hi = lo + 4 * t.numel()
        for pw in reg.values():
            if pw.lo < hi and lo < pw.hi:
                pw.stale = True


def repack_weights(dev):
    reg = _packs.get(_dev_key(dev))
    if not reg:
        return
    todo = []
    for key in list(reg):
        pw = reg[key]
        pw.unused += 1
        if pw.unused > 8:
            del reg[key]
        elif pw.stale or pw.version != pw.W._version:
            todo.append(pw)
    if todo:
        _pack_now(todo)


def drop_packs(dev):
    _packs.pop(_dev_key(dev), None)


def _x6_ok(M, N, *pairs):
    if not (GEMM_X6 & 1):
        return False
    for A, lda, K in pairs:
        if K % 4 or lda % 4 or lda < K or A.data_ptr() % 16 or M * lda >= (1 << 29):
            return False
    return True


def _x6_tn_ok(problems, K):
    if not (GEMM_X6 & 2) or len(problems) > 6:
        return False
    for pr in problems:
        A, lda, B, ldb = pr[:4]
        if len(pr) > 9 and pr[9] is not None:
            return False
        if lda % 4 or ldb % 4 or A.data_ptr() % 16 or B.data_ptr() % 16 or \
                K * max(lda, ldb) >= (1 << 29):
            return False
    return True


def gemm_w(A, lda, W, sn, sk, C, M, N, K, ldc, tag=None, stop_event=None,
           A2=None, lda2=0, W2=None, K2=0, sn2=None, sk2=None, bias=None):
    L = _L()
    p1 = packed_weight(W, N, K, sn, sk)
    p2 = packed_weight(W2, N, K2, sn if sn2 is None else sn2, sk if sk2 is None else sk2) if K2 else None
    need = _lib.ws_bytes(_lib.WS_GEMM_X6, M, N, K, K2)
    w = _lib.workspace(need, C.device, tag='gemm_x6')
    wn = w.numel()
    with _lib.timed('gemm_x6', tag):
        if stop_event is not None:
            stop_event.arm()
        check(L.danet_gemm_x6(_lib.stream(), M, N, K, ptr(_f32(A)), lda, ptr(p1),
                              K2, ptr(_f32(A2)) if K2 else None, lda2, ptr(p2) if K2 else None,
                              ptr(_f32(C)), ldc, ptr(bias), ptr(w), wn))
        if stop_event is not None:
            stop_event.attached = True
    return C


def _x6_tn_tiles(M, N):
    tail = M % 128
    rows = M - tail if (M > 128 and 1 <= tail <= 4 and N % 4 == 0) else M
    return ((rows + 127) // 128) * ((N + 127) // 128)


def gemm_group(problems, K, transA=False, transB=False, max_workgroups=0):
    L = _L()
    x6 = transA and not transB and _x6_tn_ok(problems, K)
    arr = (_lib.GemmProblem * len(problems))()
    keep = []
    for i, pr in enumerate(problems):
        A, lda, B, ldb, C, ldc, M, N, beta = pr[:9]
        bias = pr[9] if len(pr) > 9 else None
        A, B, C = _f32(A), _f32(B), _f32(C)
        keep += [A, B, C, bias]
        arr[i].A, arr[i].lda, arr[i].B, arr[i].ldb = ptr(A), lda, ptr(B), ldb
        arr[i].C, arr[i].ldc, arr[i].M, arr[i].N = ptr(C), ldc, M, N
        arr[i].bias, arr[i].beta = ptr(bias), float(beta)
    dev = problems[0][4].device
    if x6:
        need = _lib.ws_bytes(_lib.WS_GEMM_X6_TN, sum(pr[6] * pr[7] for pr in problems),
                             sum(_x6_tn_tiles(pr[6], pr[7]) for pr in problems), K)
        w = _lib.workspace(need, dev, tag='gemm_x6_tn') if need else None
        with _lib.timed('gemm_x6_tn_group'):
            check(L.danet_gemm_x6_tn_grouped(_lib.stream(), K, len(problems), arr, ptr(w),
                                             w.numel() if w is not None else 0))
        return
    w = _lib.workspace(_lib.ws_bytes(_lib.WS_GEMM_STREAMK, 0, 0, K), dev, tag='gemm_sk')
    with _lib.timed('gemm_f32_group'):
        check(L.danet_gemm_f32_streamk_grouped(_lib.stream(), int(transA), int(transB), K,
                                               len(problems), arr, int(max_workgroups),
                                               ptr(w), w.numel()))


GROUPED_DW = _lib.expert('grouped_dw', 1)
GROUPED_DW_WGS = _lib.expert('grouped_dw_wgs', 256)
GROUPED_GX = _lib.expert('grouped_gx', 512)


def colsum(A, M, N, lda, out, beta=0.0):
    L = _L()
    w, wn = _ws(_lib.ws_bytes(_lib.WS_COLSUM, M, N), out.device)
    check(L.danet_colsum_f32(_lib.stream(), M, N, ptr(_f32(A)), lda, ptr(out), float(beta),
                             ptr(w), wn))
    return out


def center(x, B, T, D, in_layout, ld_in, out, out_layout, ld_out):
    L = _L()
    scratch = torch.empty(_lib.ws_bytes(_lib.WS_CENTER_MEAN, B) // 4, dtype=torch.float32, device=x.device)
    check(L.danet_center(_lib.stream(), B, T, D, ptr(_f32(x)), in_layout, ld_in,
                         ptr(out), out_layout, ld_out, ptr(scratch)))
    return scratch[:B]


def frontend(src, want_phase=False, want_mix=False):
    assert src.is_cuda and src.dtype == torch.complex64
    src = src.contiguous()
    B, C, T, F = src.shape
    N = T * F
    dev = src.device
    out = dict(
        src_pwr=torch.empty(B, C, T, F, device=dev),
        mix_pwr=torch.empty(B, T, F, device=dev),
        mix_log=torch.empty(B, T, F, device=dev),
        phasor=torch.empty(B, T, F, 2, device=dev))
    phase = torch.empty(B, T, F, device=dev) if want_phase else None
    mix = torch.empty(B, T, F, dtype=torch.complex64, device=dev) if want_mix else None
    check(_L().danet_frontend_fwd(
        _lib.stream(), B, C, N, ptr(torch.view_as_real(src)), ptr(out['mix_pwr']),
        ptr(out['mix_log']), ptr(out['phasor']), ptr(phase), ptr(out['src_pwr']),
        ptr(torch.view_as_real(mix)) if mix is not None else None))
    if want_phase:
        out['phase'] = phase
    if want_mix:
        out['mix'] = mix
    return out


def noise_frontend(src, noise, gain=None, want_mix=False):
    assert src.is_cuda and src.dtype == torch.complex64 and src.dim() == 4 and src.is_contiguous(), \
        (src.device, src.dtype, src.shape)
    B, C, T, F = src.shape
    assert noise.dtype == torch.complex64 and noise.device == src.device and tuple(noise.shape) == (B, T, F) \
        and noise.is_contiguous(), (noise.device, noise.dtype, noise.shape)
    if gain is not None:
        assert gain.dtype == torch.float32 and gain.device == src.device and tuple(gain.shape) == (B,) \
            and gain.is_contiguous(), (gain.device, gain.dtype, gain.shape)
    dev = src.device
    out = dict(
        src_pwr=torch.empty(B, C, T, F, device=dev),
        mix_pwr=torch.empty(B, T, F, device=dev),
        mix_log=torch.empty(B, T, F, device=dev),
        phasor=torch.empty(B, T, F, 2, device=dev))
    mix = torch.empty(B, T, F, dtype=torch.complex64, device=dev) if want_mix else None
    with _lib.timed('noise_frontend'):
        _lib.noise_check(_lib.load_noise().danet_noise_frontend_fwd(
            _lib.stream(), B, C, T * F, ptr(torch.view_as_real(src)), ptr(torch.view_as_real(noise)), ptr(gain),
            ptr(out['mix_pwr']), ptr(out['mix_log']), ptr(out['phasor']), ptr(out['src_pwr']),
            ptr(torch.view_as_real(mix)) if mix is not None else None))
    if want_mix:
        out['mix'] = mix
    return out


def reattach_phase(sep_pwr, phasor, perm_idx=None):
    B, C, T, F = sep_pwr.shape
    out = torch.empty(B, C, T, F, dtype=torch.complex64, device=sep_pwr.device)
    check(_L().danet_reattach_phase(
        _lib.stream(), B, C, T * F, ptr(_f32(sep_pwr.contiguous())), ptr(phasor),
        ptr(perm_idx), ptr(torch.view_as_real(out))))
    return out


def combinations(s_data, subset_size, total_size=None, name=None):
    if total_size is None:
        total_size = s_data.shape[0]
    combs = torch.tensor(list(itertools.combinations(range(total_size), subset_size)),
                         device=s_data.device)
    return s_data[combs]


def stft(x, window, fft_size, fft_stride):
    squeeze = x.dim() == 1
    if squeeze:
        x = x[None]
    x = _f32(x.contiguous())
    n_sig, Ls = x.shape
    L = _L()
    T = L.danet_stft_num_frames(Ls, fft_size, fft_stride)
    if T < 0:
        raise ValueError('window is longer than input signal')
    F = fft_size // 2 + 1
    out = torch.empty(n_sig, T, F, dtype=torch.complex64, device=x.device)
    check(L.danet_stft(_lib.stream(), n_sig, Ls, fft_size, fft_stride, ptr(x),
                       ptr(_f32(window)), ptr(torch.view_as_real(out))))
    return out[0] if squeeze else out


def istft(X, stride, window):
    squeeze = X.dim() == 2
    if squeeze:
        X = X[None]
    assert X.dtype == torch.complex64 and X.is_cuda
    X = X.contiguous()
    n_sig, T, F = X.shape
    N = (F - 1) * 2
    L = _L()
    out = torch.empty(n_sig, T * stride, dtype=torch.float64, device=X.device)
    w, wn = _ws(_lib.ws_bytes(_lib.WS_ISTFT, n_sig, T, N, stride), X.device)
    check(L.danet_istft(_lib.stream(), n_sig, T, N, stride, ptr(torch.view_as_real(X)),
                        ptr(_f32(window)), ptr(out), ptr(w), wn))
    return out[0] if squeeze else out


PREP_DESC_DTYPE = np.dtype([('offset', '<i8'), ('length', '<i8'), ('pad_left', '<i4'), ('reserved', '<i4')])
_prep_plans = {}
_prep_plans_fast = {}


def _desc_table(who, dtype_name, desc, validate, device):
    dtype = globals()[dtype_name]
    if not torch.is_tensor(desc):
        desc = np.asarray(desc)
        if desc.dtype != dtype:
            raise TypeError('%s: desc must be a %s record array or a device tensor' % (who, dtype_name))
        validate(desc)
        desc = torch.from_numpy(np.ascontiguousarray(desc).view(np.uint8).copy()).to(device)
    row = dtype.itemsize
    assert desc.is_cuda and desc.is_contiguous() and (desc.numel() * desc.element_size()) % row == 0
    return desc, desc.numel() * desc.element_size() // row


def _c64_row_pitch(t, F):
    n_utt, t_count = t.shape[:2]
    ld = t.stride(1) if t_count > 1 else max(t.stride(1), F)
# ... 1710 lines not shown
        _fast_depth[0] -= 1
        return False


def _fast():
    return _fast_depth[0] > 0


def _grad_target(param, shape, dev):
    g = param.grad if (DIRECT_GRADS and _fast() and torch.is_tensor(param)) else None
    if g is not None and g.is_contiguous() and tuple(g.shape) == tuple(shape):
        return g, True
    return torch.empty(*shape, device=dev), False


def join_deferred():
    _flush_lazy()
    waits = {}
    while _deferred:
        main, used, _keep = _deferred.pop()
        for s in used:
            waits.setdefault((main.cuda_stream, s.cuda_stream), (main, s))
    for main, s in waits.values():
        main.wait_stream(s)


def lstm_prefill_fwd(T, B, ldy, ypads, wss):
    n = len(ypads)
    yp = (_lib.c_p * n)(*[ptr(y) for y in ypads])
    wp = (_lib.c_p * n)(*[ptr(w) for w in wss])
    check(_L().danet_lstm_fwd_prefill(_lib.stream(), T, B, ldy, n, yp, wp))


ENC_PROLOGUE = _lib.expert('enc_prologue', True)


def encoder_prologue(x, B, T, F, xc, Fp, H, ndir, ypads, fwd_wss, bwd_wss):
    n = len(ypads)
    yp = (_lib.c_p * n)(*[ptr(y) for y in ypads])
    fp = (_lib.c_p * n)(*[ptr(w) for w in fwd_wss])
    bp = (_lib.c_p * n)(*[ptr(w) for w in bwd_wss]) if bwd_wss is not None else None
    scratch = torch.empty(_lib.ws_bytes(_lib.WS_CENTER_MEAN, B) // 4, dtype=torch.float32, device=x.device)
    args = (_lib.stream(), B, T, F, ptr(_f32(x)), 0, F, ptr(xc), 1, Fp, ptr(scratch), H, ndir, ndir * H, n, yp, fp)
    rc = _L().danet_encoder_prologue(*args, bp)
    if rc == -3 and bp is not None:
        check(_L().danet_encoder_prologue(*args, None))
        return False
    check(rc)
    return True


def lstm_prefill_train(T, B, H, ndir, ypads, fwd_wss, bwd_wss):
    n = len(ypads)
    yp = (_lib.c_p * n)(*[ptr(y) for y in ypads])
    fp = (_lib.c_p * n)(*[ptr(w) for w in fwd_wss])
    bp = (_lib.c_p * n)(*[ptr(w) for w in bwd_wss])
    return _L().danet_lstm_train_prefill(_lib.stream(), T, B, H, ndir, ndir * H, n, yp, fp, bp) == 0


def lstm_layer_fwd(x, ldx, D, T, B, H, Ws, bs, x_pad_zero=False, ypad=None, ws=None):
    ndir = len(Ws)
    dev = x.device
    L = _L()
    gates = [torch.empty(T * B, 4 * H, device=dev) for _ in range(ndir)]
    cells = [torch.empty(T * B, H, device=dev) for _ in range(ndir)]
    flags = 0
    if ypad is None:
        ypad = torch.empty(T + 2, B, ndir * H, device=dev)
        ws, wn = _lstm_ws(T, B, H, ndir, dev)
    else:
        wn = ws.numel()
        flags = 1
    fused = (ldx % 4 == 0 and x.data_ptr() % 16 == 0 and (D % 4 == 0 or x_pad_zero) and
             all(W.stride(0) == 4 * H and W.stride(1) == 1 for W in Ws) and
             L.danet_lstm_fwd_fused_supported(T, B, H, ndir, D) == 1)
    if fused:
        with _lib.timed('lstm_fwd'):
            check(L.danet_lstm_fwd_fused(
                _lib.stream(), T, B, H, ndir, ptr(_f32(x)), ldx, D,
                ptr(Ws[0]), ptr(Ws[-1]), 4 * H, ptr(bs[0]), ptr(bs[-1]), ptr(ypad), ndir * H,
                ptr(gates[0]), ptr(gates[-1]), ptr(cells[0]), ptr(cells[-1]), ptr(ws), wn,
                ptr(status_word(dev)), flags))
    else:
        if _x6_ok(T * B, 4 * H, (x, ldx, D)):
            for d in range(ndir):
                gemm_w(x, ldx, Ws[d], 1, 4 * H, gates[d], T * B, 4 * H, D, 4 * H, tag='gx', bias=bs[d])
        elif GROUPED_GX and ndir == 2:
            gemm_group([(x, ldx, Ws[d], 4 * H, gates[d], 4 * H, T * B, 4 * H, 0.0, bs[d])
                        for d in range(ndir)], D, max_workgroups=GROUPED_GX)
        else:
            with _Fork(dev, ndir) as f:
                for d in range(ndir):
                    f.run(d, lambda d=d: gemm(x, Ws[d], gates[d], T * B, 4 * H, D, ldx, 4 * H,
                                              4 * H, bias=bs[d], tag='gx'))
        Whs = [W[D:] for W in Ws]
        with _lib.timed('lstm_fwd'):
            check(L.danet_lstm_fwd(
                _lib.stream(), T, B, H, ndir, ptr(gates[0]), ptr(gates[-1]),
                ptr(Whs[0]), ptr(Whs[-1]), 4 * H, ptr(ypad), ndir * H,
                ptr(gates[0]), ptr(gates[-1]), ptr(cells[0]), ptr(cells[-1]), ptr(ws), wn,
                ptr(status_word(dev)), flags))
    c = _LayerCtx()
    c.x, c.ldx, c.D, c.T, c.B, c.H, c.ndir = x, ldx, D, T, B, H, ndir
    c.ypad, c.gates, c.cells, c.Ws, c.bs = ypad, gates, cells, Ws, bs
    return c


DW_OVERLAP = _lib.expert('dw_overlap', 'auto')


def _overlap_dw(H, tn_ok=True):
    if DW_OVERLAP in ('0', '1'):
        return DW_OVERLAP == '1'
    return H <= 384 or (bool(GEMM_X6 & 2) and tn_ok)


DW_FORK_EARLY = _lib.expert('dw_fork_early', False)
BWD_DB = _lib.expert('lstm_bwd_db', True)
DB_DEFER = _lib.expert('lstm_db_defer', True)


def lstm_layer_bwd(c, dy, need_dx, layer_tag=None, is_top=False, ws_prefilled=None, dx_drop=None):
    T, B, H, D, ndir = c.T, c.B, c.H, c.D, c.ndir
    dev = dy.device
    das = [torch.empty(T * B, 4 * H, device=dev) for _ in range(ndir)]
    L = _L()
    ldy = ndir * H
    dWs, dbs, direct = [], [], []
    for d in range(ndir):
        gW, okW = _grad_target(c.Ws[d], (D + H, 4 * H), dev)
        gb, okb = _grad_target(c.bs[d], (4 * H,), dev)
        dWs.append(gW); dbs.append(gb); direct.append((okW, okb))
    dx = torch.empty(T * B, D, device=dev) if need_dx else None
    if ws_prefilled is not None:
        ws, wn = ws_prefilled, ws_prefilled.numel()
    else:
        ws, wn = _lstm_ws(T, B, H, ndir, dev)
    Whs = [W[D:] for W in c.Ws]
    b_direct = [okb for _, okb in direct]
    db_in_kernel = (BWD_DB and (all(b_direct) or not any(b_direct)) and
                    all(t.data_ptr() % 16 == 0 for t in dbs) and
                    L.danet_lstm_bwd_db_supported(T, B, H, ndir) == 1)
    def group_problems():
        probs = []
        for d in range(ndir):
            bW = 1.0 if direct[d][0] else 0.0
            hprev = c.ypad.view(-1)[(0 if d == 0 else 2 * B * ldy + H):]
            probs.append((c.x, c.ldx, das[d], 4 * H, dWs[d], 4 * H, D, 4 * H, bW))
            probs.append((hprev, ldy, das[d], 4 * H, dWs[d][D:], 4 * H, H, 4 * H, bW))
        return probs
    overlap = _overlap_dw(H, _x6_tn_ok(group_problems(), T * B))
    db_deferred = (db_in_kernel and DB_DEFER and GROUPED_DW and SIDE_STREAMS > 0 and
                   need_dx and overlap)
    with _lib.timed('lstm_bwd'):
        check(L.danet_lstm_bwd(
            _lib.stream(), T, B, H, ndir, ptr(_f32(dy)), ndir * H,
            ptr(Whs[0]), ptr(Whs[-1]), 4 * H, ptr(c.gates[0]), ptr(c.gates[-1]),
            ptr(c.cells[0]), ptr(c.cells[-1]), ptr(das[0]), ptr(das[-1]),
            ptr(dbs[0]) if db_in_kernel else None, ptr(dbs[-1]) if db_in_kernel else None,
            1.0 if all(b_direct) else 0.0, ptr(ws), wn, ptr(status_word(dev)),
            ((1 if ws_prefilled is not None else 0) | (2 if db_deferred else 0))
            if db_in_kernel else 0))

    cap = OVERLAP_GEMM_WGS if need_dx else 0

    def weight_grads(d):
        bW, bb = (1.0 if direct[d][0] else 0.0), (1.0 if direct[d][1] else 0.0)
        gemm(c.x, das[d], dWs[d], D, 4 * H, T * B, c.ldx, 4 * H, 4 * H, transA=True, beta=bW,
             max_workgroups=cap)
        hprev = c.ypad.view(-1)[(0 if d == 0 else 2 * B * ldy + H):]
        gemm(hprev, das[d], dWs[d][D:], H, 4 * H, T * B, ldy, 4 * H, 4 * H, transA=True, beta=bW,
             max_workgroups=cap)
        if not db_in_kernel:
            colsum(das[d], T * B, 4 * H, 4 * H, dbs[d], beta=bb)

    def hprev_of(d):
        return c.ypad.view(-1)[(0 if d == 0 else 2 * B * ldy + H):]

    def weight_grads_grouped(wgs=GROUPED_DW_WGS, with_bias=True):
        gemm_group(group_problems(), T * B, transA=True, max_workgroups=wgs)
        if with_bias:
            bias_grads()

    def bias_grads():
        if db_deferred:
            check(L.danet_lstm_bwd_db_reduce(_lib.stream(), T, B, H, ndir, ptr(dbs[0]), ptr(dbs[-1]),
                                             1.0 if direct[0][1] else 0.0, ptr(ws), wn))
            return
        if db_in_kernel:
            return
        for d in range(ndir):
            colsum(das[d], T * B, 4 * H, 4 * H, dbs[d], beta=1.0 if direct[d][1] else 0.0)

    fork_ev = [None]

    def input_grad(attach=False):
        if ndir == 2:
            sk = (STREAMK & 4) != 0 and (4 * H) % 16 == 0
            if _x6_ok(T * B, D, (das[0], 4 * H, 4 * H), (das[1], 4 * H, 4 * H)):
                if attach:
                    fork_ev[0] = fork_event(dev)
                gemm_w(das[0], 4 * H, c.Ws[0], 4 * H, 1, dx, T * B, D, 4 * H, D, tag='dX',
                       stop_event=fork_ev[0], A2=das[1], lda2=4 * H, W2=c.Ws[1], K2=4 * H)
                return
            if attach and sk:
                fork_ev[0] = fork_event(dev)
            gemm_kcat(das[0], 4 * H, c.Ws[0], 4 * H, 4 * H, das[1], 4 * H, c.Ws[1], 4 * H, 4 * H,
                      dx, T * B, D, D, transB=True, tag='dX', streamk=(STREAMK & 4) != 0,
                      stop_event=fork_ev[0])
            return
        for d in range(ndir):
            gemm(das[d], c.Ws[d], dx, T * B, D, 4 * H, 4 * H, 4 * H, D, transB=True,
                 beta=0.0 if d == 0 else 1.0, streamk=(STREAMK & 1) != 0, tag='dX')

    fork_early = DW_FORK_EARLY and need_dx and GROUPED_DW
    def drop_dx():
        dropout_apply(dx, dx, T * B, D, D, D, dx_drop[0], dx_drop[1])

    if need_dx and not fork_early:
        input_grad(attach=GROUPED_DW and overlap and dx_drop is None)
        if dx_drop is not None:
            drop_dx()
    hooks = bool(GRAD_READY_HOOKS) and _fast() and layer_tag is not None and \
        all(a and b for a, b in direct)
    if hooks and not need_dx:
        sides = _side_streams(dev, max(SIDE_STREAMS, 1))
        main = torch.cuda.current_stream(dev)
        for sd in sides[1:]:
            sides[0].wait_stream(sd)
        sides[0].wait_stream(main)
        with torch.cuda.stream(sides[0]):
            _fire_grad_ready(('rest',), list(c.Ws) + list(c.bs))
    with _Fork(dev, ndir + 1, defer=True, keep=(das, c.x, c.ypad, dy, ws), lazy=True,
               event=fork_ev[0], spacer=dx_drop is not None) as f:
        on_main = False
        if GROUPED_DW and not need_dx:
            if not db_in_kernel:
                f.run(1, bias_grads)
            weight_grads_grouped(wgs=512, with_bias=False)
            on_main = True
        elif GROUPED_DW and not overlap:
            weight_grads_grouped(wgs=512)
            on_main = True
        elif GROUPED_DW:
            f.run(1, weight_grads_grouped)
            if fork_early:
                input_grad()
                if dx_drop is not None:
                    drop_dx()
        else:
            for d in range(ndir):
                f.run(d + 1, lambda d=d: weight_grads(d))
        if hooks:
            f.after_all(lambda: _fire_grad_ready(('layer', layer_tag), list(c.Ws) + list(c.bs)),
                        wait_main=on_main)
    dWs = [None if direct[d][0] else dWs[d] for d in range(ndir)]
    dbs = [None if direct[d][1] else dbs[d] for d in range(ndir)]
    return dx, dWs, dbs


class LstmLayerFn(torch.autograd.Function):

    @staticmethod
    def forward(ctx, x, H, *params):
        ndir = len(params) // 2
        Ws, bs = list(params[0::2]), list(params[1::2])
        B, T, D = x.shape
        xt = x.transpose(0, 1).contiguous()
        c = lstm_layer_fwd(xt, D, D, T, B, H, Ws, bs)
        ctx.c = c
        ctx.xt = xt
        spec = _dropout_cur[0] if ndir == 2 else None
        ctx.drop = None
        if spec is not None:
            ctx.drop = (spec, spec.take())
            yd = torch.empty(T, B, 2 * H, device=x.device)
            dropout_apply(c.ypad[1:], yd, T * B, 2 * H, 2 * H, 2 * H, *ctx.drop)
            return yd.transpose(0, 1).contiguous()
        return c.ypad[1:T + 1].transpose(0, 1).contiguous()

    @staticmethod
    def backward(ctx, dy):
        c = ctx.c
        dyt = dy.transpose(0, 1).contiguous()
        if ctx.drop is not None:
            W = c.ndir * c.H
            dyt = dropout_apply(dyt, torch.empty(c.T, c.B, W, device=dy.device), c.T * c.B, W, W, W, *ctx.drop)
        dx, dWs, dbs = lstm_layer_bwd(c, dyt, ctx.needs_input_grad[0])
        join_deferred()
        out = [None, None]
        if dx is not None:
            out[0] = dx.view(c.T, c.B, c.D).transpose(0, 1).contiguous()
        for dW, db in zip(dWs, dbs):
            out += [dW, db]
        return tuple(out)


class RnnEncoderFn(torch.autograd.Function):

    @staticmethod
    def forward(ctx, x, H, L, ndir, *params):
        x = _f32(x.contiguous())
        B, T, F = x.shape
        dev = x.device
        Wout = params[-1]
        Fp = (F + 3) // 4 * 4
        xc = torch.empty(T, B, Fp, device=dev)
        ctxs = []
        cur, ld, D = xc, Fp, F
        ypads = [torch.empty(T + 2, B, ndir * H, device=dev) for _ in range(L)]
        wss = [_lstm_ws(T, B, H, ndir, dev)[0] for _ in range(L)]
        bwss = None
        if any(ctx.needs_input_grad) and BWD_DB and _L().danet_lstm_bwd_db_supported(T, B, H, ndir) == 1:
            bwss = [_lstm_ws(T, B, H, ndir, dev)[0] for _ in range(L)]
        if not ENC_PROLOGUE:
            center(x, B, T, F, 0, F, xc, 1, Fp)
            if bwss is None or not lstm_prefill_train(T, B, H, ndir, ypads, wss, bwss):
                bwss = None
                lstm_prefill_fwd(T, B, ndir * H, ypads, wss)
        else:
            if not encoder_prologue(x, B, T, F, xc, Fp, H, ndir, ypads, wss, bwss):
                bwss = None
        ctx.bwss = bwss
        spec = _dropout_cur[0] if ndir == 2 else None
        ctx.drop = (spec, spec.take(L)) if spec is not None else None
        for l in range(L):
            Ws = [params[(l * ndir + d) * 2] for d in range(ndir)]
            bs = [params[(l * ndir + d) * 2 + 1] for d in range(ndir)]
            c = lstm_layer_fwd(cur, ld, D, T, B, H, Ws, bs, x_pad_zero=True, ypad=ypads[l],
                               ws=wss[l])
            ctxs.append(c)
            cur, ld, D = c.ypad[1:], ndir * H, ndir * H
            if spec is not None:
                cur = dropout_apply(cur, torch.empty(T, B, D, device=dev), T * B, D, D, D, spec,
                                    ctx.drop[1] + l)
        yc = torch.empty(B, T, D, device=dev)
        center(cur, B, T, D, 1, D, yc, 0, D)
        O = Wout.shape[1]
        embed = torch.empty(B, T, O, device=dev)
        big = ((B * T + 127) // 128) * ((O + 127) // 128) >= 1024
        if _x6_ok(B * T, O, (yc, D, D)):
            gemm_w(yc, D, Wout, 1, O, embed, B * T, O, D, O, tag='proj')
        else:
            gemm(yc, Wout, embed, B * T, O, D, D, O, O, tag='proj',
                 streamk=(STREAMK & 2) != 0 or (big and STREAMK != 0))
        ctx.ctxs, ctx.yc, ctx.Wout = ctxs, yc, Wout
        ctx.dims = (B, T, F, H, L, ndir, D, O)
        return embed

    @staticmethod
    def backward(ctx, dembed):
        B, T, F, H, L, ndir, D, O = ctx.dims
        dembed = _f32(dembed.contiguous())
        dev = dembed.device
        dWout, direct_out = _grad_target(ctx.Wout, (D, O), dev)
        dyc = torch.empty(B, T, D, device=dev)
        x6 = _x6_ok(B * T, D, (dembed, O, O))
        ev = fork_event(dev) if ((STREAMK & 1) != 0 or x6) else None
        if x6:
            gemm_w(dembed, O, ctx.Wout, O, 1, dyc, B * T, D, O, D, tag='dYc', stop_event=ev)
        else:
            gemm(dembed, ctx.Wout, dyc, B * T, D, O, O, O, D, transB=True, streamk=(STREAMK & 1) != 0,
                 tag='dYc', stop_event=ev)
        with _Fork(dev, 2, defer=True, keep=(dembed, ctx.yc), lazy=True, event=ev) as f:
            if GROUPED_DW:
                ov = _overlap_dw(H, _x6_tn_ok([(ctx.yc, D, dembed, O, dWout, O, D, O, 0.0)], B * T))
                f.run(1 if ov else 0, lambda: gemm_group(
                    [(ctx.yc, D, dembed, O, dWout, O, D, O, 1.0 if direct_out else 0.0)], B * T,
                    transA=True, max_workgroups=GROUPED_DW_WGS if ov else 512))
            else:
                f.run(1, lambda: gemm(ctx.yc, dembed, dWout, D, O, B * T, D, O, O, transA=True,
                                      beta=1.0 if direct_out else 0.0,
                                      max_workgroups=2 * OVERLAP_GEMM_WGS, tag='dWout'))
            if GRAD_READY_HOOKS and _fast() and direct_out:
                f.after_all(lambda: _fire_grad_ready(('out',), [ctx.Wout]))
        dy = torch.empty(T, B, D, device=dev)
        center(dyc, B, T, D, 0, D, dy, 1, D)
        drop = ctx.drop
        if drop is not None:
            dropout_apply(dy, dy, T * B, D, D, D, drop[0], drop[1] + L - 1)
        grads = [None] * (2 * L * ndir)
        bwss = ctx.bwss if ctx.bwss is not None else [None] * L
        ctx.bwss = None
        for l in reversed(range(L)):
            dx, dWs, dbs = lstm_layer_bwd(ctx.ctxs[l], dy, need_dx=(l > 0), layer_tag=l,
                                          is_top=(l == L - 1), ws_prefilled=bwss[l],
                                          dx_drop=(drop[0], drop[1] + l - 1) if (drop is not None and l > 0)
                                          else None)
            for d in range(ndir):
                grads[(l * ndir + d) * 2] = dWs[d]
                grads[(l * ndir + d) * 2 + 1] = dbs[d]
            dy = dx
# ... 599 lines not shown
        return out, masks

    @staticmethod
    def backward(ctx, dout, _dmasks):
        if dout is None:
            return None, None, None, None, None
        mix_pwr, attr, embed_flat = ctx.saved_tensors
        act, B, C, N, E = ctx.args
        dev = dout.device
        dembed = torch.empty(B, N, E, device=dev)
        dattr = torch.empty(B, C, E, device=dev)
        L = _L()
        w, wn = _ws(_lib.ws_bytes(_lib.WS_SEPARATE_BWD, B, C, N, E), dev)
        check(L.danet_separate_bwd(_lib.stream(), act, B, C, N, E, ptr(mix_pwr), ptr(attr),
                                   ptr(embed_flat), ptr(_f32(dout.contiguous())), ptr(dembed),
                                   ptr(dattr), ptr(w), wn))
        if ctx.token is not None and ctx.token.share and ctx.needs_input_grad[1]:
            ctx.token.dembed = dembed
        return None, dattr, dembed, None, None


class PitMseFn(torch.autograd.Function):

    @staticmethod
    def forward(ctx, src, sep_pwr, phasor, mode, eps):
        assert src.dtype == torch.complex64
        B, C, T, F = sep_pwr.shape
        N = T * F
        dev = sep_pwr.device
        src = src.contiguous()
        sep_pwr = _f32(sep_pwr.contiguous())
        phasor = _f32(phasor.contiguous())
        loss, snr = torch.empty((), device=dev), torch.empty((), device=dev)
        perm_idx = torch.empty(B, dtype=torch.int32, device=dev)
        L = _L()
        w, wn = _ws(_lib.ws_bytes(_lib.WS_PIT_MSE, B, C, N), dev)
        check(L.danet_pit_mse_fwd(_lib.stream(), mode, B, C, N, ptr(torch.view_as_real(src)),
                                  ptr(sep_pwr), ptr(phasor), eps, ptr(loss), ptr(snr),
                                  ptr(perm_idx), ptr(w), wn))
        ctx.save_for_backward(src, sep_pwr, phasor, perm_idx)
        ctx.args = (mode, B, C, N)
        ctx.mark_non_differentiable(snr, perm_idx)
        ctx.set_materialize_grads(False)
        return loss, snr, perm_idx

    @staticmethod
    def backward(ctx, dloss, _dsnr, _dperm):
        src, sep_pwr, phasor, perm_idx = ctx.saved_tensors
        mode, B, C, N = ctx.args
        if dloss is None:
            return None, None, None, None, None
        dsep = torch.empty_like(sep_pwr)
        check(_L().danet_pit_mse_bwd(_lib.stream(), mode, B, C, N,
                                     ptr(torch.view_as_real(src)), ptr(sep_pwr), ptr(phasor),
                                     ptr(perm_idx), 1.0, ptr(_f32(dloss.contiguous())), ptr(dsep)))
        return None, dsep, None, None, None


class SeparatePitFn(torch.autograd.Function):

    @staticmethod
    def forward(ctx, mix_pwr, attr, embed_flat, src, phasor, act, mode, eps):
        assert src.dtype == torch.complex64
        B, T, F = mix_pwr.shape
        C, E = attr.shape[1], attr.shape[2]
        N = T * F
        dev = mix_pwr.device
        mix_pwr = _f32(mix_pwr.contiguous())
        attr_c = _f32(attr.contiguous())
        embed_flat = _f32(embed_flat.contiguous())
        src = src.contiguous()
        phasor = _f32(phasor.contiguous())
        loss, snr = torch.empty((), device=dev), torch.empty((), device=dev)
        perm_idx = torch.empty(B, dtype=torch.int32, device=dev)
        L = _L()
        records = torch.empty(_lib.ws_bytes(_lib.WS_SEPARATE_PIT_RECORDS, B, N) // 4, device=dev)
        tok = getattr(attr, '_danet_dembed_token', None)
        gpart = None
        if (HEADS_GRADFWD and HEADS_RECOMPUTE and _chain() and tok is not None and
                tok.kind in ('anchor', 'truth') and ctx.needs_input_grad[1] and ctx.needs_input_grad[2] and
                tok.same_inputs(embed_flat, mix_pwr)):
            nb = _lib.ws_bytes(_lib.WS_SEPARATE_PIT_GRAD, B, C, N, E)
            if nb:
                gpart = torch.empty(nb // 4, device=dev)
        check(L.danet_separate_pit_fwd_records(
            _lib.stream(), act, mode, B, C, N, E, ptr(mix_pwr), ptr(attr_c), ptr(embed_flat),
            ptr(torch.view_as_real(src)), ptr(phasor), None, ptr(records), ptr(gpart)))
        ctx.gpart = gpart

        def final():
            check(L.danet_separate_pit_final(_lib.stream(), B, C, N, eps, ptr(records), ptr(loss),
                                             ptr(snr), ptr(perm_idx)))
        if _chain():
            _on_side(dev, final, keep=(records, loss, snr, perm_idx))
        else:
            final()
        ctx.records = records
        ctx.save_for_backward(mix_pwr, attr_c, embed_flat, src, phasor, perm_idx)
        ctx.args = (act, mode, B, C, N, E)
        ctx.token = getattr(attr, '_danet_dembed_token', None)
        ctx.mark_non_differentiable(snr, perm_idx)
        ctx.set_materialize_grads(False)
        return loss, snr, perm_idx

    @staticmethod
    def backward(ctx, dloss, _dsnr, _dperm):
        if dloss is None:
            return (None,) * 8
        mix_pwr, attr, embed_flat, src, phasor, perm_idx = ctx.saved_tensors
        act, mode, B, C, N, E = ctx.args
        records, ctx.records = ctx.records, None
        gpart, ctx.gpart = ctx.gpart, None
        dev = dloss.device
        tok = ctx.token
        defer = (HEADS_RECOMPUTE and _chain() and tok is not None and tok.kind in ('anchor', 'truth') and
                 ctx.needs_input_grad[1] and ctx.needs_input_grad[2] and
                 tok.same_inputs(embed_flat, mix_pwr))
        dembed = None if defer else torch.empty(B, N, E, device=dev)
        dattr = torch.empty(B, C, E, device=dev)
        dl = _f32(dloss.contiguous())
        L = _L()
        if defer and gpart is not None:
            tok.recipe = (act, mode, mix_pwr, src, phasor, records, dl, gpart)
            return None, dattr, None, None, None, None, None, None
        w, wn = _ws(_lib.ws_bytes(_lib.WS_SEPARATE_PIT, B, C, N, E), dev)
        check(L.danet_separate_pit_bwd(_lib.stream(), act, mode, B, C, N, E, ptr(mix_pwr),
                                       ptr(attr), ptr(embed_flat), ptr(torch.view_as_real(src)),
                                       ptr(phasor), None, ptr(records), 1.0,
                                       ptr(dl), ptr(dembed), ptr(dattr), ptr(w), wn))
        if defer:
            tok.recipe = (act, mode, mix_pwr, src, phasor, records, dl, None)
            return None, dattr, None, None, None, None, None, None
        if ctx.token is not None and ctx.token.share and ctx.needs_input_grad[1]:
            ctx.token.dembed = dembed
        return None, dattr, dembed, None, None, None, None, None


def separate_pit_loss(s_mix_pwr, s_attractors, s_embed_flat, s_x, phasor, act, mode=0, eps=1e-7):
    C = s_attractors.shape[1]
    loss, snr, idx = SeparatePitFn.apply(s_mix_pwr, s_attractors, s_embed_flat, s_x, phasor,
                                         act, mode, eps)
    v_perms = torch.tensor(list(itertools.permutations(range(C))), dtype=torch.int32)
    return loss, v_perms, idx, snr


def pit_mse_loss(s_x, s_y_pwr, phasor, mode=0, eps=1e-7):
    C = s_y_pwr.shape[1]
    loss, snr, idx = PitMseFn.apply(s_x, s_y_pwr, phasor, mode, eps)
    v_perms = torch.tensor(list(itertools.permutations(range(C))), dtype=torch.int32)
    return loss, v_perms, idx, snr


def adam_clip_step(theta, grad, m, v, lr_t, beta1=0.9, beta2=0.999, eps=1e-8, clip=100.0,
                   grad_scale=1.0, zero_grad=False):
    check(_L().danet_adam_clip_step(_lib.stream(), theta.numel(), ptr(_f32(theta)),
                                    ptr(_f32(grad)), ptr(_f32(m)), ptr(_f32(v)), lr_t, beta1,
                                    beta2, eps, clip if clip else 0.0, grad_scale,
                                    int(bool(zero_grad))))
    weights_written(theta)


def gclip_partials(n):
    p = _lib.load_gclip().danet_gclip_partials(int(n))
    if p <= 0:
        _lib.gclip_check(-1)
    return p


def grad_sumsq(grad, partials=None):
    n = grad.numel()
    if partials is None:
        partials = torch.empty(gclip_partials(n), dtype=torch.float64, device=grad.device)
    assert partials.is_cuda and partials.dtype == torch.float64 and partials.is_contiguous(), partials.dtype
    _lib.gclip_check(_lib.load_gclip().danet_gclip_sumsq(_lib.stream(), n, ptr(_f32(grad)), ptr(partials),
                                                         partials.numel()))
    return partials


def adam_gclip_step(theta, grad, m, v, lr_t, beta1=0.9, beta2=0.999, eps=1e-8, clip=100.0,
                    grad_scale=1.0, zero_grad=False, max_norm=None, partials=None, norm_out=None):
    assert norm_out.is_cuda and norm_out.dtype == torch.float64 and norm_out.numel() == 2
    assert partials.is_cuda and partials.dtype == torch.float64
    _lib.gclip_check(_lib.load_gclip().danet_gclip_adam_step(
        _lib.stream(), theta.numel(), ptr(_f32(theta)), ptr(_f32(grad)), ptr(_f32(m)), ptr(_f32(v)), lr_t, beta1,
        beta2, eps, clip if clip else 0.0, grad_scale, int(bool(zero_grad)), float(max_norm), ptr(partials),
        partials.numel(), ptr(norm_out)))
    weights_written(theta)
```

danet-tensorflow_amd/ozers.py:

```python
import math

import torch

from .hparams import hparams
from . import ops


class _FlatOptimizer(object):
    def __init__(self, learn_rate):
        self.learn_rate = learn_rate
        self.theta = self.grad = None

    def bind(self, theta, grad):
        self.theta, self.grad = theta, grad


class TfAdam(_FlatOptimizer):
    def __init__(self, learn_rate, beta1=0.9, beta2=0.999, epsilon=1e-8):
        super(TfAdam, self).__init__(learn_rate)
        self.beta1, self.beta2, self.epsilon = beta1, beta2, epsilon
        self.m = self.v = None

    def bind(self, theta, grad):
        super(TfAdam, self).bind(theta, grad)
        self.m = torch.zeros_like(theta)
        self.v = torch.zeros_like(theta)

    def step(self, t, lr, clip=None, grad_scale=1.0, zero_grad=False, ranges=None, max_norm=None, partials=None,
             norm_out=None):
        lr_t = lr * math.sqrt(1. - self.beta2 ** t) / (1. - self.beta1 ** t)
        if max_norm is not None:
            assert ranges is None, 'a global-norm clip cannot be issued in pieces'
            if partials is None:
                partials = ops.grad_sumsq(self.grad)
            if norm_out is None:
                norm_out = torch.empty(2, dtype=torch.float64, device=self.grad.device)
            ops.adam_gclip_step(self.theta, self.grad, self.m, self.v, lr_t, self.beta1, self.beta2, self.epsilon,
                                clip or 0.0, grad_scale, zero_grad, max_norm, partials, norm_out)
            return
        for lo, hi in (ranges if ranges is not None else [(0, self.theta.numel())]):
            ops.adam_clip_step(self.theta[lo:hi], self.grad[lo:hi], self.m[lo:hi], self.v[lo:hi],
                               lr_t, self.beta1, self.beta2, self.epsilon, clip or 0.0,
                               grad_scale, zero_grad)


class TfSgd(_FlatOptimizer):
    def step(self, t, lr, clip=None, grad_scale=1.0, zero_grad=False, ranges=None, max_norm=None, partials=None,
             norm_out=None):
        if max_norm is not None:
            assert ranges is None, 'a global-norm clip cannot be issued in pieces'
            if partials is None:
                partials = ops.grad_sumsq(self.grad)
            norm = partials.sum().sqrt() * abs(grad_scale)
            lim = norm + 1e-6
            coef = torch.where(lim > max_norm, max_norm / lim, torch.ones_like(lim))
            if norm_out is not None:
                norm_out[0], norm_out[1] = norm, coef
            g = self.grad * (coef * grad_scale).to(torch.float32)
            if clip:
                g = g.clamp_(-clip, clip)
            self.theta.add_(g, alpha=-lr)
            if zero_grad:
                self.grad.zero_()
            return
        for lo, hi in (ranges if ranges is not None else [(0, self.theta.numel())]):
            g = self.grad[lo:hi] * grad_scale
            if clip:
                g = g.clamp_(-clip, clip)
            self.theta[lo:hi].add_(g, alpha=-lr)
            if zero_grad:
                self.grad[lo:hi].zero_()


@hparams.register_optimizer('sgd')
def sgd_ozer(learn_rate, lr_decay=None, lr_decay_epoch=2, **kwargs):
    return TfSgd(learn_rate)


@hparams.register_optimizer('adam')
def adam_ozer(learn_rate, lr_decay=None, lr_decay_epoch=2, **kwargs):
    return TfAdam(learn_rate, **kwargs)
```

include/danet_hip.h:

```cpp
#ifndef DANET_HIP_H
#define DANET_HIP_H

#include <stddef.h>
#include <stdint.h>

#ifdef __cplusplus
extern "C" {
#endif
#pragma GCC visibility push(default)

#define DANET_OK 0
#define DANET_ERR_ARG (-1)
#define DANET_ERR_LAUNCH (-2)
#define DANET_ERR_UNSUPPORTED (-3)
#define DANET_ERR_WORKSPACE (-4)

#define DANET_ABI_VERSION 7

typedef void* danet_stream_t;

int danet_abi_version(void);
const char* danet_last_error(void);

int danet_set_option(const char* name, int value);
int danet_get_option(const char* name, int* value);
void danet_reset_options(void);
int danet_option_count(void);
const char* danet_option_name(int index);

enum {
  DANET_WS_ISTFT = 0,
  DANET_WS_GEMM,
  DANET_WS_GEMM_STREAMK,
  DANET_WS_COLSUM,
  DANET_WS_LSTM,
  DANET_WS_ATTRACTOR_TRUTH,
  DANET_WS_ATTRACTOR_ANCHOR,
  DANET_WS_SEPARATE_BWD,
  DANET_WS_SEPARATE_PIT,
  DANET_WS_SEPARATE_PIT_RECORDS,
  DANET_WS_PIT_MSE,
  DANET_WS_CENTER_MEAN,
  DANET_WS_GEMM_X6,
  DANET_WS_GEMM_PACK,
  DANET_WS_GEMM_X6_TN,
  DANET_WS_SEPARATE_PIT_GRAD,
  DANET_WS_COUNT
};
size_t danet_workspace_bytes(int op, const int64_t* dims, int n_dims);

int danet_stft_num_frames(int64_t Ls, int N, int S);
int danet_stft(danet_stream_t stream, int n_sig, int64_t Ls, int N, int S,
               const float* x, const float* window, float* out_c64);

int danet_istft(danet_stream_t stream, int n_sig, int T, int N, int S,
                const float* X_c64, const float* window, double* out,
                void* ws, size_t ws_bytes);

int danet_frontend_fwd(danet_stream_t stream, int B, int C, int64_t N,
                       const float* src_c64, float* mix_pwr, float* mix_log,
                       float* phasor, float* phase, float* src_pwr,
                       float* mix_c64);

int danet_reattach_phase(danet_stream_t stream, int B, int C, int64_t N,
                         const float* sep_pwr, const float* phasor,
                         const int32_t* perm_idx, float* out_c64);

int danet_center(danet_stream_t stream, int B, int T, int D,
                 const float* in, int in_layout, int ld_in,
                 float* out, int out_layout, int ld_out, float* mean);

int danet_gemm_f32(danet_stream_t stream, int transA, int transB,
                   int M, int N, int K,
                   const float* A, int lda, const float* B, int ldb,
                   float* C, int ldc, const float* bias, float beta,
                   void* ws, size_t ws_bytes, int max_workgroups);

int danet_gemm_f32_streamk(danet_stream_t stream, int transA, int transB,
                           int M, int N, int K,
                           const float* A, int lda, const float* B, int ldb,
                           float* C, int ldc, const float* bias, float beta,
                           void* ws, size_t ws_bytes);
typedef struct {
  const float* A; int lda;
  const float* B; int ldb;
  float* C; int ldc;
  int M, N;
  const float* bias;
  float beta;
} danet_gemm_problem_t;
int danet_gemm_f32_streamk_grouped(danet_stream_t stream, int transA, int transB,
                                   int K, int nprob, const danet_gemm_problem_t* probs,
                                   int max_workgroups, void* ws, size_t ws_bytes);
int danet_gemm_f32_streamk_kcat(danet_stream_t stream, int transA, int transB, int M, int N,
                                int K1, const float* A1, int lda1, const float* B1, int ldb1,
                                int K2, const float* A2, int lda2, const float* B2, int ldb2,
                                float* C, int ldc, const float* bias, float beta,
                                void* ws, size_t ws_bytes);

typedef struct {
  const float* src; long long stride_n, stride_k;
  int N, K;
  void* out; size_t out_bytes;
} danet_gemm_pack_t;
int danet_gemm_pack_weights(danet_stream_t stream, int n, const danet_gemm_pack_t* jobs);
int danet_gemm_x6(danet_stream_t stream, int M, int N,
                  int K1, const float* A1, int lda1, const void* B1_packed,
                  int K2, const float* A2, int lda2, const void* B2_packed,
                  float* C, int ldc, const float* bias, void* ws, size_t ws_bytes);

int danet_gemm_x6_tn_grouped(danet_stream_t stream, int K, int nprob, const danet_gemm_problem_t* probs,
                             void* ws, size_t ws_bytes);

int danet_next_launch_events(void* start, void* stop);
int danet_event_create(void** event);
int danet_event_destroy(void* event);
int danet_stream_wait_event(danet_stream_t stream, void* event);

int danet_colsum_f32(danet_stream_t stream, int M, int N, const float* A,
                     int lda, float* out, float beta, void* ws,
                     size_t ws_bytes);

#define DANET_STATUS_TIMEOUT 0x3F800000
int danet_lstm_fwd(danet_stream_t stream, int T, int B, int H, int ndir,
                   const float* gx_f, const float* gx_b,
                   const float* Wh_f, const float* Wh_b, int ldw,
                   float* ypad, int ldy,
                   float* gates_f, float* gates_b,
                   float* cell_f, float* cell_b,
                   void* ws, size_t ws_bytes, int32_t* status, int flags);

#define DANET_LSTM_PREFILLED 1
#define DANET_LSTM_DB_DEFERRED 2
int danet_lstm_fwd_prefill(danet_stream_t stream, int T, int B, int ldy, int n,
                           float* const* ypads, void* const* wss );
int danet_lstm_train_prefill(danet_stream_t stream, int T, int B, int H, int ndir, int ldy, int n,
                             float* const* ypads, void* const* fwd_wss ,
                             void* const* bwd_wss );
int danet_encoder_prologue(danet_stream_t stream, int B, int T, int D, const float* in, int in_layout,
                           int ld_in, float* out, int out_layout, int ld_out, float* mean,
                           int H, int ndir, int ldy, int n, float* const* ypads,
                           void* const* fwd_wss , void* const* bwd_wss );

int danet_lstm_fwd_fused_supported(int T, int B, int H, int ndir, int D);
int danet_lstm_fwd_fused(danet_stream_t stream, int T, int B, int H, int ndir,
                         const float* x, int ldx, int D,
                         const float* W_f, const float* W_b, int ldw,
                         const float* bias_f, const float* bias_b,
                         float* ypad, int ldy,
                         float* gates_f, float* gates_b,
                         float* cell_f, float* cell_b,
                         void* ws, size_t ws_bytes, int32_t* status, int flags);

int danet_lstm_bwd_db_supported(int T, int B, int H, int ndir);
int danet_lstm_bwd(danet_stream_t stream, int T, int B, int H, int ndir,
                   const float* dy, int lddy,
                   const float* Wh_f, const float* Wh_b, int ldw,
                   const float* gates_f, const float* gates_b,
                   const float* cell_f, const float* cell_b,
                   float* da_f, float* da_b, float* db_f, float* db_b, float beta,
                   void* ws, size_t ws_bytes, int32_t* status, int flags);
int danet_lstm_bwd_db_reduce(danet_stream_t stream, int T, int B, int H, int ndir,
                             float* db_f, float* db_b, float beta, const void* ws, size_t ws_bytes);

int danet_attractor_truth_fwd(danet_stream_t stream, int mode, int B, int C,
                              int64_t N, int E, const float* embed,
                              const float* src_pwr, const float* mix_pwr,
                              float eps, float* attr, float* denom,
                              void* ws, size_t ws_bytes);
int danet_attractor_truth_bwd(danet_stream_t stream, int mode, int B, int C,
                              int64_t N, int E, const float* dattr,
                              const float* src_pwr, const float* mix_pwr,
                              const float* denom, float eps, float* dembed);
int danet_attractor_truth_bwd_sep(danet_stream_t stream, int tmode, int B, int C, int64_t N, int E,
                                  const float* dattr, const float* src_pwr, const float* mix_pwr,
                                  const float* denom, float eps, const float* embed,
                                  const float* attr, int act, int mode, const float* src_c64,
                                  const float* phasor, const int32_t* perm_idx,
                                  const float* records, float dloss, const float* dloss_dev,
                                  float* dembed, const float* dattr_partials );

int danet_attractor_anchor_fwd(danet_stream_t stream, int B, int C, int64_t N,
                               int E, int A, const float* embed,
                               const float* anchors, float* attr,
                               float* asets, float* asum, int32_t* choice,
                               void* ws, size_t ws_bytes);
int danet_attractor_anchor_bwd_embed(danet_stream_t stream, int B, int C, int64_t N, int E, int A,
                                     const float* dattr, const float* embed, const float* anchors,
                                     const float* attr, const float* asum, const int32_t* choice,
                                     float* dembed, void* ws, size_t ws_bytes);
int danet_attractor_anchor_bwd_embed_sep(danet_stream_t stream, int B, int C, int64_t N, int E, int A,
                                         const float* dattr, const float* embed, const float* anchors,
                                         const float* attr, const float* asum, const int32_t* choice,
                                         int act, int mode, const float* mix_pwr, const float* src_c64,
                                         const float* phasor, const int32_t* perm_idx,
                                         const float* records, float dloss, const float* dloss_dev,
                                         float* dembed, void* ws, size_t ws_bytes,
                                         const float* dattr_partials );
int danet_attractor_anchor_bwd_anchors(danet_stream_t stream, int B, int C, int64_t N, int E, int A,
// ... 49 lines not shown
```

Baseline: 14220 mixture-seconds/s.

## Fold split-K weight-grad and bias-grad partial reductions into the Adam step

The grouped split-K weight-gradient GEMM for the first LSTM layer (no dx needed) and the in-kernel bias-gradient partials can now leave their per-slice partial sums in workspace instead of running a separate reduce kernel. A new Adam kernel takes a table of up to 8 gradient segments, sums the slices while it updates theta, m and v, and writes the summed gradient back unless grad is zeroed. This removes the reduction launches and one write-then-read pass over those gradients. In exchange the Adam kernel does per-element segment lookups and more strided reads, and the workspace must stay alive until the optimizer step.

After: 14270 mixture-seconds/s (median of 6 runs). No clear change (+0.3%).

```diff
diff --git a/danet-tensorflow_amd/_build.py b/danet-tensorflow_amd/_build.py
--- a/danet-tensorflow_amd/_build.py
+++ b/danet-tensorflow_amd/_build.py
@@ -52,7 +52,8 @@
 PHASE = _extension('phase', *_shared('ext_core', 'wave_metric'))
 ONLINE = _extension('online', *_shared('ext_core'))
 CAUSAL = _extension('causal', *_shared('ext_core'))
-MORE_EXTENSIONS = (STITCH, BSS, STOI, PHASE, ONLINE, CAUSAL)
+GRADSEG = _extension('gradseg', *_shared('ext_core', 'adam_one'))
+MORE_EXTENSIONS = (STITCH, BSS, STOI, PHASE, ONLINE, CAUSAL, GRADSEG)
 METRIC_LIB = METRIC.out
 NOISE_LIB = NOISE.out
 LEVEL_LIB = LEVEL.out
@@ -66,6 +67,7 @@
 PHASE_LIB = PHASE.out
 ONLINE_LIB = ONLINE.out
 CAUSAL_LIB = CAUSAL.out
+GRADSEG_LIB = GRADSEG.out
 
 
 def _sources(src_dir):
@@ -208,6 +210,10 @@
     return _build_spec(CAUSAL, force, verbose)
 
 
+def build_gradseg(force=False, verbose=True):
+    return _build_spec(GRADSEG, force, verbose)
+
+
 def build_variant(name, defs):
     out = os.path.join(CSRC, 'libdanet_hip_%s.so' % name)
     res = _compile_all(CSRC, os.path.join(CSRC, 'build_' + name), True, 0.0, defs)
diff --git a/danet-tensorflow_amd/_lib.py b/danet-tensorflow_amd/_lib.py
--- a/danet-tensorflow_amd/_lib.py
+++ b/danet-tensorflow_amd/_lib.py
@@ -279,6 +279,20 @@
     'danet_causal_project': (c_int, [c_p, c_int, c_int, c_int, c_p, c_int, c_p, c_int, c_p, c_int]),
 }
 
+class GradSegment(ctypes.Structure):
+    _fields_ = [('first', c_i64), ('length', c_i64), ('slab', c_p), ('slice_stride', c_i64),
+                ('slices', ctypes.c_int32), ('from_zero', ctypes.c_int32), ('beta', c_f32),
+                ('reserved', ctypes.c_int32)]
+
+
+GRADSEG_MAX_SEGMENTS = 8
+GRADSEG_PROTOTYPES = {
+    'danet_gradseg_abi_version': (c_int, []),
+    'danet_gradseg_last_error': (ctypes.c_char_p, []),
+    'danet_gradseg_adam_step': (c_int, [c_p, c_i64, c_p, c_p, c_p, c_p, c_f32, c_f32, c_f32, c_f32, c_f32, c_f32,
+                                        c_int, c_int, ctypes.POINTER(GradSegment)]),
+}
+
 Library = collections.namedtuple('Library', 'name so path_var handle_var prototypes abi prefix needs')
 CONV_ABI_VERSION = DROPOUT_ABI_VERSION = PREP_ABI_VERSION = MIX_ABI_VERSION = SPEED_ABI_VERSION = 1
 REVERB_ABI_VERSION = 1
@@ -341,7 +355,11 @@
 CAUSAL = Library('causal', 'libdanet_causal_hip.so', 'CAUSAL_LIB_PATH', '_causal', CAUSAL_PROTOTYPES,
                  CAUSAL_ABI_VERSION, 'danet_causal_', 'the lstm-causal encoder and streaming inference need the HIP '
                  'extension library')
-MORE_EXTENSIONS = (STITCH, BSS, STOI, PHASE, ONLINE, CAUSAL)
+GRADSEG_ABI_VERSION = 1
+GRADSEG = Library('gradseg', 'libdanet_gradseg_hip.so', 'GRADSEG_LIB_PATH', '_gradseg', GRADSEG_PROTOTYPES,
+                  GRADSEG_ABI_VERSION, 'danet_gradseg_', 'the optimizer launch with gradient segments needs the HIP '
+                  'extension library')
+MORE_EXTENSIONS = (STITCH, BSS, STOI, PHASE, ONLINE, CAUSAL, GRADSEG)
 
 LIB_PATH = os.environ.get('DANET_LIB_PATH') or os.path.join(_CSRC, CORE.so)
 CONV_LIB_PATH = os.path.join(_CSRC, CONV.so)
@@ -363,8 +381,9 @@
 PHASE_LIB_PATH = os.path.join(_CSRC, PHASE.so)
 ONLINE_LIB_PATH = os.path.join(_CSRC, ONLINE.so)
 CAUSAL_LIB_PATH = os.path.join(_CSRC, CAUSAL.so)
+GRADSEG_LIB_PATH = os.path.join(_CSRC, GRADSEG.so)
 _lib = _conv = _dropout = _prep = _mix = _speed = _reverb = _metric = _noise = _level = _wavloss = _gclip = _dpcl = None
-_neval = _stitch = _bss = _stoi = _phase = _online = _causal = None
+_neval = _stitch = _bss = _stoi = _phase = _online = _causal = _gradseg = None
 _lock = threading.Lock()
 
 
@@ -625,6 +644,17 @@
         _check(CAUSAL, rc)
 
 
+def load_gradseg():
+    if _gradseg is not None:
+        return _gradseg
+    return _load(GRADSEG)
+
+
+def gradseg_check(rc):
+    if rc != 0:
+        _check(GRADSEG, rc)
+
+
 _expert = None
 _expert_seen = set()
 
@@ -687,7 +717,7 @@
 
 (WS_ISTFT, WS_GEMM, WS_GEMM_STREAMK, WS_COLSUM, WS_LSTM, WS_ATTRACTOR_TRUTH, WS_ATTRACTOR_ANCHOR,
  WS_SEPARATE_BWD, WS_SEPARATE_PIT, WS_SEPARATE_PIT_RECORDS, WS_PIT_MSE, WS_CENTER_MEAN,
- WS_GEMM_X6, WS_GEMM_PACK, WS_GEMM_X6_TN, WS_SEPARATE_PIT_GRAD) = range(16)
+ WS_GEMM_X6, WS_GEMM_PACK, WS_GEMM_X6_TN, WS_SEPARATE_PIT_GRAD, WS_LSTM_DB_PARTIALS) = range(17)
 
 
 def ws_bytes(op, *dims):
diff --git a/danet-tensorflow_amd/csrc/gemm_x6.hip b/danet-tensorflow_amd/csrc/gemm_x6.hip
--- a/danet-tensorflow_amd/csrc/gemm_x6.hip
+++ b/danet-tensorflow_amd/csrc/gemm_x6.hip
@@ -925,6 +925,7 @@
 
 __global__ __launch_bounds__(256) void gemm_x6_tn_reduce_kernel(X6TArgs g) {
   const X6TProblem& q = g.p[blockIdx.y];
+  if (!q.C) return;
   const int M = q.M, N = q.N, ldc = q.ldc;
   const float beta = q.beta;
   const float* __restrict__ slab = g.slab + q.slab_off;
@@ -962,9 +963,12 @@
   int tiles = 0;
   long long sum_mn = 0;
   bool slicable = true, ragged = false;
+  int kept = 0;
   for (int i = 0; i < nprob; ++i) {
     const danet_gemm_problem_t& q = probs[i];
-    DANET_CHECK_ARG(q.M > 0 && q.N > 0 && q.A && q.B && q.C, "gemm_x6_tn: bad problem %d", i);
+    DANET_CHECK_ARG(q.M > 0 && q.N > 0 && q.A && q.B, "gemm_x6_tn: bad problem %d", i);
+    DANET_CHECK_ARG(q.C || q.ldc == q.N, "gemm_x6_tn: problem %d keeps its slices (C == NULL): ldc must be N", i);
+    kept += q.C ? 0 : 1;
     DANET_CHECK_ARG(q.bias == nullptr && (q.beta == 0.f || q.beta == 1.f), "gemm_x6_tn: no bias; beta 0 or 1");
     DANET_CHECK_ARG(q.lda >= q.M && q.ldb >= q.N && q.ldc >= q.N, "gemm_x6_tn: leading dimension too small");
     if (q.lda % 4 || q.ldb % 4 || ((((uintptr_t)q.A | (uintptr_t)q.B)) & 15) != 0) {
@@ -988,6 +992,11 @@
   for (int i = nprob; i < X6T_MAX_PROBLEMS; ++i) g.p[i] = g.p[0];
   g.nprob = nprob; g.K = K; g.tiles = tiles;
   int s = slicable ? x6t_splitk(tiles, K) : 1;
+  if (kept && s == 1) {
+    danet_set_error("gemm_x6_tn: a problem keeps its slices (C == NULL), but this launch has one K slice "
+                    "(DANET_WS_GEMM_X6_TN answers 0 for it: pass C)");
+    return DANET_ERR_UNSUPPORTED;
+  }
   g.splitk = s;
   g.slab_stride = sum_mn;
   g.slab = (float*)ws;
@@ -1011,9 +1020,10 @@
     gemm_x6_tn_kernel<false><<<grid, block, X6T_SMEM_BYTES, stream>>>(g);
   }
   DANET_CHECK_LAUNCH();
-  if (s > 1) {
+  if (s > 1 && kept < nprob) {
     long long most = 0;
-    for (int i = 0; i < nprob; ++i) most = max(most, (long long)probs[i].M * probs[i].N / 4);
+    for (int i = 0; i < nprob; ++i)
+      if (probs[i].C) most = max(most, (long long)probs[i].M * probs[i].N / 4);
     dim3 rgrid((unsigned)min((long long)1024, (most + 255) / 256), (unsigned)nprob);
     gemm_x6_tn_reduce_kernel<<<rgrid, block, 0, stream>>>(g);
     DANET_CHECK_LAUNCH();
diff --git a/danet-tensorflow_amd/csrc/gradseg/gradseg.hip b/danet-tensorflow_amd/csrc/gradseg/gradseg.hip
--- /dev/null
+++ b/danet-tensorflow_amd/csrc/gradseg/gradseg.hip
@@ -0,0 +1,119 @@
+#include <hip/hip_runtime.h>
+#include <math.h>
+#include <string.h>
+
+#include "danet_gradseg_hip.h"
+#define DANET_EXT gradseg
+#define DANET_EXT_UPPER GRADSEG
+#include "ext_core.h"
+#include "adam_one.h"
+
+static inline int64_t cdiv64(int64_t a, int64_t b) { return (a + b - 1) / b; }
+
+struct SegTable {
+  danet_gradseg_t s[DANET_GRADSEG_MAX_SEGMENTS];
+  int64_t lo, hi;
+  int n;
+};
+
+__global__ __launch_bounds__(256) void gradseg_adam_kernel(
+    int64_t n, float* __restrict__ theta, float* __restrict__ grad, float* __restrict__ m,
+    float* __restrict__ v, float lr_t, float b1, float b2, float eps, float clip, float gscale,
+    int zero_grad, SegTable tab) {
+  const int64_t n4 = n / 4;
+  const int64_t stride = (int64_t)gridDim.x * blockDim.x;
+  const int64_t t0 = (int64_t)blockIdx.x * blockDim.x + threadIdx.x;
+  for (int64_t i = t0; i < n4; i += stride) {
+    const int64_t e = i * 4;
+    const float* slab = nullptr;
+    int64_t sstride = 0;
+    int slices = 0, from_zero = 0;
+    float beta = 0.f;
+    if (e >= tab.lo && e < tab.hi) {
+#pragma unroll
+      for (int k = 0; k < DANET_GRADSEG_MAX_SEGMENTS; ++k) {
+        const int64_t j = e - tab.s[k].first;
+        if (k < tab.n && j >= 0 && j < tab.s[k].length) {
+          slab = tab.s[k].slab + j;
+          sstride = tab.s[k].slice_stride;
+          slices = tab.s[k].slices;
+          from_zero = tab.s[k].from_zero;
+          beta = tab.s[k].beta;
+        }
+      }
+    }
+    f32x4 th = reinterpret_cast<f32x4*>(theta)[i];
+    f32x4 mi = reinterpret_cast<f32x4*>(m)[i], vi = reinterpret_cast<f32x4*>(v)[i];
+    f32x4 g;
+    if (slab) {
+      f32x4 p[8];
+#pragma unroll
+      for (int z = 0; z < 8; ++z)
+        if (z < slices) p[z] = *reinterpret_cast<const f32x4*>(slab + (size_t)z * sstride);
+      f32x4 g0 = {0.f, 0.f, 0.f, 0.f};
+      if (beta != 0.f) g0 = reinterpret_cast<f32x4*>(grad)[i];
+      g = p[0];
+      if (from_zero) g = (f32x4){0.f, 0.f, 0.f, 0.f} + g;
+#pragma unroll
+      for (int z = 1; z < 8; ++z)
+        if (z < slices) g += p[z];
+      for (int z = 8; z < slices; ++z) g += *reinterpret_cast<const f32x4*>(slab + (size_t)z * sstride);
+      if (beta != 0.f) g += g0;
+    } else {
+      g = reinterpret_cast<f32x4*>(grad)[i];
+    }
+    const f32x4 gsum = g;
+#pragma unroll
+    for (int c = 0; c < 4; ++c) {
+      float t_ = th[c], g_ = g[c], m_ = mi[c], v_ = vi[c];
+      adam_one(t_, g_, m_, v_, lr_t, b1, b2, eps, clip, gscale);
+      th[c] = t_; mi[c] = m_; vi[c] = v_;
+    }
+    reinterpret_cast<f32x4*>(theta)[i] = th;
+    reinterpret_cast<f32x4*>(m)[i] = mi;
+    reinterpret_cast<f32x4*>(v)[i] = vi;
+    if (zero_grad) reinterpret_cast<f32x4*>(grad)[i] = (f32x4){0.f, 0.f, 0.f, 0.f};
+    else if (slab) reinterpret_cast<f32x4*>(grad)[i] = gsum;
+  }
+  for (int64_t i = n4 * 4 + t0; i < n; i += stride) {
+    float th = theta[i], g = grad[i], mi = m[i], vi = v[i];
+    adam_one(th, g, mi, vi, lr_t, b1, b2, eps, clip, gscale);
+    theta[i] = th; m[i] = mi; v[i] = vi;
+    if (zero_grad) grad[i] = 0.f;
+  }
+}
+
+extern "C" int danet_gradseg_adam_step(void* stream, int64_t n, float* theta, float* grad, float* m, float* v,
+                                       float lr_t, float beta1, float beta2, float eps, float clip,
+                                       float grad_scale, int zero_grad, int n_segments,
+                                       const danet_gradseg_t* segments) {
+  CHECK_ARG(n >= 1, "adam_step: n must be >= 1 (got %lld)", (long long)n);
+  CHECK_ARG(theta && grad && m && v, "adam_step: null pointer");
+  CHECK_ARG((((uintptr_t)theta | (uintptr_t)grad | (uintptr_t)m | (uintptr_t)v) & 15) == 0,
+            "adam_step: theta, grad, m, v must be 16-byte aligned");
+  CHECK_ARG(n_segments >= 0 && n_segments <= DANET_GRADSEG_MAX_SEGMENTS && (n_segments == 0 || segments),
+            "adam_step: 0..%d segments (got %d)", DANET_GRADSEG_MAX_SEGMENTS, n_segments);
+  SegTable tab;
+  memset(&tab, 0, sizeof(tab));
+  tab.n = n_segments;
+  int64_t end = 0;
+  for (int k = 0; k < n_segments; ++k) {
+    const danet_gradseg_t& s = segments[k];
+    CHECK_ARG(s.first >= end && s.first % 4 == 0 && s.length > 0 && s.length % 4 == 0 && s.length <= n - s.first,
+              "adam_step: segment %d [%lld, +%lld) must be a multiple of 4 in both, inside [0, %lld) and behind "
+              "the segment before it", k, (long long)s.first, (long long)s.length, (long long)n);
+    CHECK_ARG(s.slab && ((uintptr_t)s.slab & 15) == 0, "adam_step: segment %d: slab null or not 16-byte aligned", k);
+    CHECK_ARG(s.slices >= 1 && (s.slices == 1 || (s.slice_stride >= s.length && s.slice_stride % 4 == 0)),
+              "adam_step: segment %d: %d slices with stride %lld (a multiple of 4, >= length)", k, s.slices,
+              (long long)s.slice_stride);
+    CHECK_ARG((s.beta == 0.f || s.beta == 1.f) && s.reserved == 0, "adam_step: segment %d: beta must be 0 or 1", k);
+    tab.s[k] = s;
+    end = s.first + s.length;
+  }
+  if (n_segments) { tab.lo = segments[0].first; tab.hi = end; }
+  const int grid = (int)min((int64_t)2048, cdiv64(cdiv64(n, 4), 256));
+  gradseg_adam_kernel<<<grid, 256, 0, (hipStream_t)stream>>>(n, theta, grad, m, v, lr_t, beta1, beta2, eps, clip,
+                                                             grad_scale, zero_grad, tab);
+  CHECK_LAUNCH();
+  return DANET_GRADSEG_OK;
+}
diff --git a/danet-tensorflow_amd/csrc/lstm.hip b/danet-tensorflow_amd/csrc/lstm.hip
--- a/danet-tensorflow_amd/csrc/lstm.hip
+++ b/danet-tensorflow_amd/csrc/lstm.hip
@@ -1373,6 +1373,12 @@
   return align_up(ring_offset(T) + ring, 256) + align_up((size_t)ndir * cdiv(B, 16) * 4 * H * sizeof(float), 256);
 }
 
+size_t dn_ws_lstm_db_partials(int T, int B, int H, int ndir) {
+  if (T <= 0 || B <= 0 || H <= 0 || H % 4 != 0 || (ndir != 1 && ndir != 2)) return 0;
+  const RsPlan rs = choose_rs_plan(B, H, ndir);
+  return rs.ok ? align_up(ring_offset(T) + rs.ring_bytes, 256) : 0;
+}
+
 static int lstm_check_common(int T, int B, int H, int ndir, void* ws, size_t ws_bytes) {
   DANET_CHECK_ARG(T > 0 && B > 0 && H > 0, "lstm: non-positive shape");
   DANET_CHECK_ARG(ndir == 1 || ndir == 2, "lstm: ndir must be 1 or 2");
diff --git a/danet-tensorflow_amd/csrc/workspace.cpp b/danet-tensorflow_amd/csrc/workspace.cpp
--- a/danet-tensorflow_amd/csrc/workspace.cpp
+++ b/danet-tensorflow_amd/csrc/workspace.cpp
@@ -20,9 +20,10 @@
 size_t dn_ws_gemm_pack(int N, int K);
 size_t dn_ws_gemm_x6_tn(long long sum_mn, int tiles, int K);
 size_t dn_ws_separate_pit_grad(int B, int C, int64_t N, int E);
+size_t dn_ws_lstm_db_partials(int T, int B, int H, int ndir);
 
 extern "C" size_t danet_workspace_bytes(int op, const int64_t* d, int n) {
-  static const int kDims[DANET_WS_COUNT] = {4, 3, 3, 2, 4, 4, 5, 4, 4, 2, 3, 1, 4, 2, 3, 4};
+  static const int kDims[DANET_WS_COUNT] = {4, 3, 3, 2, 4, 4, 5, 4, 4, 2, 3, 1, 4, 2, 3, 4, 4};
   if (op < 0 || op >= DANET_WS_COUNT || !d || n != kDims[op]) {
     danet_set_error("workspace_bytes: op %d takes %d dims, got %d", op,
                     (op >= 0 && op < DANET_WS_COUNT) ? kDims[op] : -1, n);
@@ -53,6 +54,7 @@
     case DANET_WS_GEMM_PACK: return dn_ws_gemm_pack((int)d[0], (int)d[1]);
     case DANET_WS_GEMM_X6_TN: return dn_ws_gemm_x6_tn((long long)d[0], (int)d[1], (int)d[2]);
     case DANET_WS_SEPARATE_PIT_GRAD: return dn_ws_separate_pit_grad((int)d[0], (int)d[1], d[2], (int)d[3]);
+    case DANET_WS_LSTM_DB_PARTIALS: return dn_ws_lstm_db_partials((int)d[0], (int)d[1], (int)d[2], (int)d[3]);
   }
   return (size_t)-1;
 }
diff --git a/danet-tensorflow_amd/model.py b/danet-tensorflow_amd/model.py
--- a/danet-tensorflow_amd/model.py
+++ b/danet-tensorflow_amd/model.py
@@ -550,6 +550,10 @@
             ops.drop_lazy(self.device)
             raise
         self._early, self._in_step = None, True
+        segments = None
+        if (self.grad_clip_norm is None and not self._early_adam and not dist.is_dist() and self._buckets is None
+                and getattr(self.ozer, 'takes_segments', False) and self.ozer.grad is self._flat_grad):
+            ops.grad_segments_begin(self._flat_grad)
         self._grads_clean = False
         try:
             with ops.fast_backward():
@@ -562,6 +566,7 @@
                         self._grad_store if dist.is_dist() else self._flat_grad)
         finally:
             self._in_step = False
+            segments = ops.grad_segments_end()
             chain.__exit__(None, None, None)
             ops.join_deferred()
         self.step_count += 1
@@ -573,7 +578,8 @@
         norm_out = None
         if self.grad_clip_norm is None:
             self.ozer.step(self.step_count, self.learn_rate, clip=hparams.GRAD_CLIP_THRES,
-                           grad_scale=grad_scale, zero_grad=not self.keep_grads, ranges=ranges)
+                           grad_scale=grad_scale, zero_grad=not self.keep_grads, ranges=ranges,
+                           **(dict(segments=segments) if segments is not None else {}))
         else:
             self._gclip_partials = ops.grad_sumsq(self._flat_grad, self._gclip_partials)
             norm_out = torch.empty(2, dtype=torch.float64, device=self.device)
diff --git a/danet-tensorflow_amd/ops.py b/danet-tensorflow_amd/ops.py
--- a/danet-tensorflow_amd/ops.py
+++ b/danet-tensorflow_amd/ops.py
@@ -192,7 +192,51 @@
     return ((rows + 127) // 128) * ((N + 127) // 128)
 
 
-def gemm_group(problems, K, transA=False, transB=False, max_workgroups=0):
+ADAM_SEGMENTS = _lib.expert('adam_segments', True)
+
+
+class GradSegments(object):
+    def __init__(self, grad):
+        self.grad, self.segs, self.keep = grad, [], []
+
+    def room(self, k):
+        return len(self.segs) + k <= _lib.GRADSEG_MAX_SEGMENTS
+
+    def takes(self, t, numel=None):
+        n = t.numel() if numel is None else numel
+        lo, hi = self.grad.data_ptr(), self.grad.data_ptr() + 4 * self.grad.numel()
+        return (t.is_contiguous() and t.dtype == torch.float32 and 0 < n <= t.numel() and lo <= t.data_ptr() and
+                t.data_ptr() + 4 * n <= hi and (t.data_ptr() - lo) % 16 == 0 and n % 4 == 0)
+
+    def add(self, t, slab, slice_stride, slices, beta, from_zero=False, keep=(), numel=None):
+        assert self.takes(t, numel) and self.room(1) and slab % 16 == 0
+        self.segs.append((t.data_ptr(), t.numel() if numel is None else numel, int(slab), int(slice_stride),
+                          int(slices), float(beta), int(bool(from_zero))))
+        self.keep += list(keep)
+
+    def table(self, grad):
+        arr = (_lib.GradSegment * len(self.segs))()
+        for i, (p, n, slab, st, s, beta, fz) in enumerate(sorted(self.segs)):
+            first = (p - grad.data_ptr()) // 4
+            assert 0 <= first and first + n <= grad.numel(), 'segment outside the buffer the optimizer steps'
+            arr[i].first, arr[i].length, arr[i].slab, arr[i].slice_stride = first, n, slab, st
+            arr[i].slices, arr[i].from_zero, arr[i].beta, arr[i].reserved = s, fz, beta, 0
+        return arr, len(self.segs)
+
+
+_grad_segments = [None]
+
+
+def grad_segments_begin(flat_grad):
+    _grad_segments[0] = GradSegments(flat_grad) if (ADAM_SEGMENTS and flat_grad.data_ptr() % 16 == 0) else None
+
+
+def grad_segments_end():
+    gs, _grad_segments[0] = _grad_segments[0], None
+    return gs if gs is not None and gs.segs else None
+
+
+def gemm_group(problems, K, transA=False, transB=False, max_workgroups=0, keep_slices=None):
     L = _L()
     x6 = transA and not transB and _x6_tn_ok(problems, K)
     arr = (_lib.GemmProblem * len(problems))()
@@ -207,9 +251,20 @@
         arr[i].bias, arr[i].beta = ptr(bias), float(beta)
     dev = problems[0][4].device
     if x6:
-        need = _lib.ws_bytes(_lib.WS_GEMM_X6_TN, sum(pr[6] * pr[7] for pr in problems),
-                             sum(_x6_tn_tiles(pr[6], pr[7]) for pr in problems), K)
-        w = _lib.workspace(need, dev, tag='gemm_x6_tn') if need else None
+        sum_mn = sum(pr[6] * pr[7] for pr in problems)
+        need = _lib.ws_bytes(_lib.WS_GEMM_X6_TN, sum_mn, sum(_x6_tn_tiles(pr[6], pr[7]) for pr in problems), K)
+        gs = keep_slices
+        if gs is not None and need and gs.room(len(problems)) and all(
+                pr[5] == pr[7] and gs.takes(pr[4], pr[6] * pr[7]) for pr in problems):
+            w = _lib.workspace(need, dev, tag='gemm_x6_tn_kept')
+            off = 0
+            for i, pr in enumerate(problems):
+                arr[i].C = None
+                gs.add(pr[4], w.data_ptr() + 4 * off, sum_mn, need // (4 * sum_mn), pr[8], keep=(w,),
+                       numel=pr[6] * pr[7])
+                off += pr[6] * pr[7]
+        else:
+            w = _lib.workspace(need, dev, tag='gemm_x6_tn') if need else None
         with _lib.timed('gemm_x6_tn_group'):
             check(L.danet_gemm_x6_tn_grouped(_lib.stream(), K, len(problems), arr, ptr(w),
                                              w.numel() if w is not None else 0))
@@ -2226,6 +2281,13 @@
     overlap = _overlap_dw(H, _x6_tn_ok(group_problems(), T * B))
     db_deferred = (db_in_kernel and DB_DEFER and GROUPED_DW and SIDE_STREAMS > 0 and
                    need_dx and overlap)
+    gs = _grad_segments[0] if (GROUPED_DW and not need_dx) else None
+    db_off = 0
+    if (gs is not None and db_in_kernel and all(b_direct) and gs.room(ndir) and all(gs.takes(t) for t in dbs)):
+        db_off = _lib.ws_bytes(_lib.WS_LSTM_DB_PARTIALS, T, B, H, ndir)
+        if (ptr(ws) + db_off) % 16:
+            db_off = 0
+    db_segments = db_off > 0
     with _lib.timed('lstm_bwd'):
         check(L.danet_lstm_bwd(
             _lib.stream(), T, B, H, ndir, ptr(_f32(dy)), ndir * H,
@@ -2233,8 +2295,12 @@
             ptr(c.cells[0]), ptr(c.cells[-1]), ptr(das[0]), ptr(das[-1]),
             ptr(dbs[0]) if db_in_kernel else None, ptr(dbs[-1]) if db_in_kernel else None,
             1.0 if all(b_direct) else 0.0, ptr(ws), wn, ptr(status_word(dev)),
-            ((1 if ws_prefilled is not None else 0) | (2 if db_deferred else 0))
+            ((1 if ws_prefilled is not None else 0) | (2 if (db_deferred or db_segments) else 0))
             if db_in_kernel else 0))
+    if db_segments:
+        G = (B + 15) // 16
+        for d in range(ndir):
+            gs.add(dbs[d], ptr(ws) + db_off + d * G * 4 * H * 4, 4 * H, G, 1.0, from_zero=True, keep=(ws,))
 
     cap = OVERLAP_GEMM_WGS if need_dx else 0
 
@@ -2251,8 +2317,8 @@
     def hprev_of(d):
         return c.ypad.view(-1)[(0 if d == 0 else 2 * B * ldy + H):]
 
-    def weight_grads_grouped(wgs=GROUPED_DW_WGS, with_bias=True):
-        gemm_group(group_problems(), T * B, transA=True, max_workgroups=wgs)
+    def weight_grads_grouped(wgs=GROUPED_DW_WGS, with_bias=True, keep_slices=None):
+        gemm_group(group_problems(), T * B, transA=True, max_workgroups=wgs, keep_slices=keep_slices)
         if with_bias:
             bias_grads()
 
@@ -2311,7 +2377,7 @@
         if GROUPED_DW and not need_dx:
             if not db_in_kernel:
                 f.run(1, bias_grads)
-            weight_grads_grouped(wgs=512, with_bias=False)
+            weight_grads_grouped(wgs=512, with_bias=False, keep_slices=gs if all(okW for okW, _ in direct) else None)
             on_main = True
         elif GROUPED_DW and not overlap:
             weight_grads_grouped(wgs=512)
@@ -3217,7 +3283,14 @@
 
 
 def adam_clip_step(theta, grad, m, v, lr_t, beta1=0.9, beta2=0.999, eps=1e-8, clip=100.0,
-                   grad_scale=1.0, zero_grad=False):
+                   grad_scale=1.0, zero_grad=False, segments=None):
+    if segments is not None:
+        arr, n = segments.table(grad)
+        _lib.gradseg_check(_lib.load_gradseg().danet_gradseg_adam_step(
+            _lib.stream(), theta.numel(), ptr(_f32(theta)), ptr(_f32(grad)), ptr(_f32(m)), ptr(_f32(v)), lr_t, beta1,
+            beta2, eps, clip if clip else 0.0, grad_scale, int(bool(zero_grad)), n, arr))
+        weights_written(theta)
+        return
     check(_L().danet_adam_clip_step(_lib.stream(), theta.numel(), ptr(_f32(theta)),
                                     ptr(_f32(grad)), ptr(_f32(m)), ptr(_f32(v)), lr_t, beta1,
                                     beta2, eps, clip if clip else 0.0, grad_scale,
diff --git a/danet-tensorflow_amd/ozers.py b/danet-tensorflow_amd/ozers.py
--- a/danet-tensorflow_amd/ozers.py
+++ b/danet-tensorflow_amd/ozers.py
@@ -16,6 +16,8 @@
 
 
 class TfAdam(_FlatOptimizer):
+    takes_segments = True
+
     def __init__(self, learn_rate, beta1=0.9, beta2=0.999, epsilon=1e-8):
         super(TfAdam, self).__init__(learn_rate)
         self.beta1, self.beta2, self.epsilon = beta1, beta2, epsilon
@@ -27,8 +29,13 @@
         self.v = torch.zeros_like(theta)
 
     def step(self, t, lr, clip=None, grad_scale=1.0, zero_grad=False, ranges=None, max_norm=None, partials=None,
-             norm_out=None):
+             norm_out=None, segments=None):
         lr_t = lr * math.sqrt(1. - self.beta2 ** t) / (1. - self.beta1 ** t)
+        if segments is not None:
+            assert ranges is None and max_norm is None, 'gradient segments need the whole buffer and no norm clip'
+            ops.adam_clip_step(self.theta, self.grad, self.m, self.v, lr_t, self.beta1, self.beta2, self.epsilon,
+                               clip or 0.0, grad_scale, zero_grad, segments=segments)
+            return
         if max_norm is not None:
             assert ranges is None, 'a global-norm clip cannot be issued in pieces'
             if partials is None:
diff --git a/include/danet_gradseg_hip.h b/include/danet_gradseg_hip.h
--- /dev/null
+++ b/include/danet_gradseg_hip.h
@@ -0,0 +1,42 @@
+#ifndef DANET_GRADSEG_HIP_H
+#define DANET_GRADSEG_HIP_H
+
+#include <stddef.h>
+#include <stdint.h>
+
+#ifdef __cplusplus
+extern "C" {
+#endif
+#pragma GCC visibility push(default)
+
+#define DANET_GRADSEG_ABI_VERSION 1
+
+#define DANET_GRADSEG_OK 0
+#define DANET_GRADSEG_ERR_ARG (-1)
+#define DANET_GRADSEG_ERR_LAUNCH (-2)
+
+#define DANET_GRADSEG_MAX_SEGMENTS 8
+
+typedef struct {
+  int64_t first;
+  int64_t length;
+  const float* slab;
+  int64_t slice_stride;
+  int32_t slices;
+  int32_t from_zero;
+  float beta;
+  int32_t reserved;
+} danet_gradseg_t;
+
+int danet_gradseg_abi_version(void);
+const char* danet_gradseg_last_error(void);
+
+int danet_gradseg_adam_step(void* stream, int64_t n, float* theta, float* grad, float* m, float* v, float lr_t,
+                            float beta1, float beta2, float eps, float clip, float grad_scale, int zero_grad,
+                            int n_segments, const danet_gradseg_t* segments );
+
+#pragma GCC visibility pop
+#ifdef __cplusplus
+}
+#endif
+#endif
diff --git a/include/danet_hip.h b/include/danet_hip.h
--- a/include/danet_hip.h
+++ b/include/danet_hip.h
@@ -45,6 +45,7 @@
   DANET_WS_GEMM_PACK,
   DANET_WS_GEMM_X6_TN,
   DANET_WS_SEPARATE_PIT_GRAD,
+  DANET_WS_LSTM_DB_PARTIALS,
   DANET_WS_COUNT
 };
 size_t danet_workspace_bytes(int op, const int64_t* dims, int n_dims);
```
